# openGemini/openGemini

Hardware: NVIDIA H100
Metric: decoded+aggregated rows/s (higher is better)
Workload: dtype f64

## Files before the change

opengemini_b200/csrc/agg_kernels.cuh:

```cuda
#pragma once
#include "agg_ops.cuh"
#include "decode.cuh"
#include "internal.h"

namespace ogpu {

#define OG_NO_BUCKET 0xFFFFFFFFu

struct DirP {
    const uint8_t *data;
    const uint64_t *page_off;
    const uint32_t *page_len;
    const uint32_t *seg_series, *seg_rows, *series_seg_begin;
    const int64_t *seg_tmin, *seg_tmax;
    uint32_t n_segments, n_columns;
};

struct ChunkP {
    uint32_t series_begin, series_end;
    uint32_t seg_begin, seg_end;
    Tri cells[OG_MAX_CALLS];
    uint32_t nb;
    Tri edges[OG_MAX_CALLS];
    uint32_t *edge_bucket;
    Tri gcells[OG_MAX_CALLS];
    uint32_t gc_cols, gc_tail0, gc_edge0, gc_col0;
    uint32_t J;
    int *err;
    int *flags;
};

__device__ __forceinline__ size_t cell_idx(const ChunkP &ch, uint32_t series, uint32_t b) { return (size_t)(series - ch.series_begin) * ch.nb + b; }

__device__ __forceinline__ void report_err(int *err, int code, uint32_t seg) {
    if (atomicCAS(&err[0], 0, code) == 0) err[1] = (int)seg;
}

__device__ __forceinline__ void store_part(const Tri &a, size_t i, const Part &p) {
    a.val[i] = p.v; a.ok[i] = (uint8_t)p.ok;
    if (a.tim) a.tim[i] = p.t;
}
__device__ __forceinline__ Part load_part(const Tri &a, size_t i) {
    Part p; p.ok = a.ok[i]; p.v = a.val[i]; p.t = a.tim ? a.tim[i] : 0; return p;
}
__device__ __forceinline__ void store_cell(const ChunkP &ch, int call, uint32_t series, uint32_t b, const Part &p) {
    store_part(ch.cells[call], cell_idx(ch, series, b), p);
    ch.flags[0] = 1;
}

struct SegWindows {
    const QueryP &q; const ChunkP &ch;
    const uint32_t seg; const size_t e; const uint32_t series;
    uint32_t cur_b = OG_NO_BUCKET, head_b = OG_NO_BUCKET; bool head_done = false;
    int64_t we = 0;

    __device__ __forceinline__ SegWindows(const QueryP &q_, const ChunkP &ch_, uint32_t seg_, size_t e_, uint32_t series_)
        : q(q_), ch(ch_), seg(seg_), e(e_), series(series_) {}
    template <int NC> __device__ __forceinline__ void flush(const Part (&parts)[NC], bool final) {
        if (cur_b == OG_NO_BUCKET) return;
#pragma unroll
        for (int c = 0; c < NC; c++) {
            if (!head_done) store_part(ch.edges[c], e, parts[c]);
            else if (final) store_part(ch.edges[c], e + 1, parts[c]);
            else if (parts[c].ok) store_cell(ch, c, series, cur_b, parts[c]);
        }
        if (!head_done) { head_done = true; head_b = cur_b; }
    }
    template <int NC> __device__ __forceinline__ bool enter(int64_t t, Part (&parts)[NC]) {
        if (cur_b != OG_NO_BUCKET && t < we) return true;
        flush(parts, false);
        cur_b = bucket_of(t, q.start, q.interval);
        if (cur_b >= q.n_buckets) { report_err(ch.err, D_CORRUPT, seg); cur_b = OG_NO_BUCKET; return false; }
        we = q.start + (int64_t)(cur_b + 1) * q.interval;
#pragma unroll
        for (int c = 0; c < NC; c++) parts[c] = part_empty();
        return true;
    }
    template <int NC> __device__ __forceinline__ void end(const Part (&parts)[NC]) {
        const uint32_t last_b = cur_b;
        const bool single = !head_done;
        flush(parts, true);
        ch.edge_bucket[e] = head_b;
        ch.edge_bucket[e + 1] = (single || head_b == OG_NO_BUCKET) ? OG_NO_BUCKET : last_b;
        if (head_b != OG_NO_BUCKET) ch.flags[1] = 1;
    }
};

__global__ void k_validate(DirP d, const int32_t *col_types, uint32_t *seg_rows, unsigned long long *totals ,
                           uint32_t *max_rows, int *err) {
    uint32_t seg = blockIdx.x * blockDim.x + threadIdx.x;
    if (seg >= d.n_segments) return;
    size_t ti = (size_t)d.n_columns * d.n_segments + seg;
    TimeDesc t;
    int rc = parse_time_page(d.data + d.page_off[ti], d.page_len[ti], t);
    if (rc == D_OK && t.rows == 0) rc = D_CORRUPT;
    if (rc == D_OK) {
        int64_t last = t.t0; bool unsorted = false;
        if (t.kind == 0) last = (int64_t)((uint64_t)t.t0 + (uint64_t)(t.rows - 1) * t.delta);
        else {
            TimeIter it; it.init(t);
            for (uint32_t i = 0; i < t.rows; i++) { const int64_t x = it.next(); unsorted |= x < last; last = x; }
            it.finish(); rc = it.err;
        }
        if (rc == D_OK && (t.t0 < d.seg_tmin[seg] || last > d.seg_tmax[seg] || last < t.t0 || unsorted)) rc = D_CORRUPT;
    }
    if (rc != D_OK) { report_err(err, rc, seg); seg_rows[seg] = 0; return; }
    seg_rows[seg] = t.rows;
    unsigned long long bytes = d.page_len[ti];
    for (uint32_t c = 0; c < d.n_columns; c++) {
        size_t pi = (size_t)c * d.n_segments + seg;
        uint32_t len = d.page_len[pi];
        if (len == 0) continue;
        bytes += len;
        PageHdr h;
        rc = parse_field_header(d.data + d.page_off[pi], len, col_types[c], t.rows, h);
        if (rc == D_OK && h.rows != t.rows) rc = D_CORRUPT;
        if (rc == D_OK && h.bitmap && hdr_valid_rows(h) != h.rows - h.nil_count) rc = D_CORRUPT;
        if (rc == D_OK && !h.one_row && h.nil_count < h.rows) {
            if (h.block_len < 1) rc = D_CORRUPT;
            else {
                int tag = __ldg(h.block) >> 4, ty = col_types[c];
                if (ty == OG_TYPE_FLOAT) rc = (tag == 0 || tag == 3 || tag == 4 || tag == 5) ? D_OK : (tag == 1 || tag == 2 || tag == 6) ? D_UNSUPPORTED : D_CORRUPT;
                else if (ty == OG_TYPE_INT) rc = (tag == 1 || tag == 2 || tag == 4) ? D_OK : tag == 3 ? D_UNSUPPORTED : D_CORRUPT;
                else if (ty == OG_TYPE_BOOL) rc = tag == 1 ? D_OK : D_CORRUPT;
                else if (ty == OG_TYPE_STRING) rc = D_OK;
                else rc = D_UNSUPPORTED;
            }
        }
        if (rc != D_OK) { report_err(err, rc, seg); return; }
    }
    atomicAdd(&totals[0], (unsigned long long)t.rows);
    atomicAdd(&totals[1], bytes);
    atomicMax(max_rows, t.rows);
    if (t.kind != 0 && t.kind != 3) atomicAdd(&totals[2], 1ull);
}

__global__ void k_fill_seg_series(const uint32_t *series_seg_begin, uint32_t n_series, uint32_t *seg_series) {
    uint32_t s = blockIdx.x;
    if (s >= n_series) return;
    for (uint32_t g = series_seg_begin[s] + threadIdx.x; g < series_seg_begin[s + 1]; g += blockDim.x) seg_series[g] = s;
}

struct TileP {
    uint32_t tile_begin, tile_end, R;
    uint32_t S;
    uint64_t *vals[OG_MAX_COLS];
    uint8_t *okb[OG_MAX_COLS];
    int64_t *times;
    uint8_t *keep;
};

__global__ void k_decode_tile(DirP d, QueryP q, TileP tp, int *err) {
    uint32_t seg = tp.tile_begin + blockIdx.x * blockDim.x + threadIdx.x;
    if (seg >= tp.tile_end) return;
    uint32_t slot = blockIdx.y;
    const size_t base = seg - tp.tile_begin, S = tp.S;
    uint32_t rows = d.seg_rows[seg];
    if (slot == q.n_cols) {
        size_t ti = (size_t)d.n_columns * d.n_segments + seg;
        TimeDesc t;
        int rc = parse_time_page(d.data + d.page_off[ti], d.page_len[ti], t);
        if (rc == D_OK) {
            TimeIter it; it.init(t);
            for (uint32_t i = 0; i < t.rows; i++) tp.times[base + i * S] = it.next();
            it.finish(); rc = it.err;
        }
        if (rc != D_OK) report_err(err, rc, seg);
        return;
    }
    size_t pi = (size_t)q.col_index[slot] * d.n_segments + seg;
    uint64_t *out = tp.vals[slot] + base; uint8_t *okb = tp.okb[slot] + base;
    ColIter it;
    it.init(d.data + d.page_off[pi], d.page_len[pi], q.col_type[slot], rows);
    for (uint32_t i = 0; i < rows; i++) { uint64_t v = 0; okb[i * S] = it.next(v); out[i * S] = v; }
    it.finish();
    if (it.err != D_OK) report_err(err, it.err, seg);
}

__device__ __forceinline__ bool term_pass(const FilterP &f, uint64_t raw) {
    if (f.type == OG_TYPE_FLOAT || (f.type == OG_TYPE_INT && f.const_is_float)) {
        double v = f.type == OG_TYPE_FLOAT ? u2d(raw) : (double)(int64_t)raw;
        double c = f.const_is_float ? f.fval : (double)f.ival;
        switch (f.op) {
        case OG_OP_LT: return !(v >= c);
        case OG_OP_LTE: return !(v > c);
        case OG_OP_GT: return !(v <= c);
        case OG_OP_GTE: return !(v < c);
        case OG_OP_EQ: return !(v != c);
        default: return !(v == c);
        }
    }
    int64_t v = f.type == OG_TYPE_BOOL ? (int64_t)(raw != 0) : (int64_t)raw, c = f.ival;
    switch (f.op) {
    case OG_OP_LT: return !(v >= c);
    case OG_OP_LTE: return !(v > c);
    case OG_OP_GT: return !(v <= c);
    case OG_OP_GTE: return !(v < c);
    case OG_OP_EQ: return !(v != c);
    default: return !(v == c);
    }
}

__global__ void k_filter_tile(DirP d, QueryP q, TileP tp) {
    size_t idx = (size_t)blockIdx.x * blockDim.x + threadIdx.x;
    size_t total = (size_t)tp.S * tp.R;
    if (idx >= total) return;
    uint32_t row = (uint32_t)(idx / tp.S), sl = (uint32_t)(idx % tp.S);
    if (sl >= tp.tile_end - tp.tile_begin) return;
    if (row >= d.seg_rows[tp.tile_begin + sl]) { tp.keep[idx] = 0; return; }
    int64_t t = tp.times[idx];
    bool keep = t >= q.tmin && t <= q.tmax;
    if (keep && q.n_filter) {
        uint32_t stack = 0; int sp = 0;
        for (uint32_t i = 0; i < q.n_filter; i++) {
            const FilterP &f = q.filter[i];
            if (f.kind == OG_F_TERM) {
                bool pass = tp.okb[f.col_slot][idx] && term_pass(f, tp.vals[f.col_slot][idx]);
                stack |= (uint32_t)pass << sp; sp++;
            } else {
                uint32_t b = (stack >> (sp - 1)) & 1, a = (stack >> (sp - 2)) & 1;
                uint32_t r = f.kind == OG_F_AND ? (a & b) : (a | b);
                sp -= 2; stack &= ~(3u << sp); stack |= r << sp; sp++;
            }
        }
        keep = stack & 1;
    }
    tp.keep[idx] = keep;
}

__global__ void k_window_reduce(DirP d, QueryP q, TileP tp, ChunkP ch) {
    uint32_t sl = blockIdx.x * blockDim.x + threadIdx.x;
    uint32_t seg = tp.tile_begin + sl;
    if (seg >= tp.tile_end) return;
    const uint32_t rows = d.seg_rows[seg], series = d.seg_series[seg];
    const size_t S = tp.S, e = 2 * (size_t)(seg - ch.seg_begin);
    Part parts[OG_MAX_CALLS];
    uint32_t cur_b = OG_NO_BUCKET, head_b = OG_NO_BUCKET; bool head_done = false;
    int64_t we = 0;
    auto flush = [&](bool final) {
        if (cur_b == OG_NO_BUCKET) return;
        for (uint32_t c = 0; c < q.n_calls; c++) {
            if (!head_done) store_part(ch.edges[c], e, parts[c]);
            else if (final) store_part(ch.edges[c], e + 1, parts[c]);
            else if (parts[c].ok) store_cell(ch, (int)c, series, cur_b, parts[c]);
        }
        if (!head_done) { head_done = true; head_b = cur_b; }
    };
    for (uint32_t r = 0; r < rows; r++) {
        const size_t ix = (size_t)r * S + sl;
        const int64_t t = tp.times[ix];
        if (t < q.tmin) continue;
        if (t > q.tmax) break;
        if (cur_b == OG_NO_BUCKET || t >= we) {
            flush(false);
            cur_b = bucket_of(t, q.start, q.interval);
            if (cur_b >= q.n_buckets) { report_err(ch.err, D_CORRUPT, seg); cur_b = OG_NO_BUCKET; break; }
            we = q.start + (int64_t)(cur_b + 1) * q.interval;
#pragma unroll
            for (uint32_t c = 0; c < OG_MAX_CALLS; c++) parts[c] = part_empty();
        }
        if (!tp.keep[ix]) continue;
#pragma unroll
        for (uint32_t c = 0; c < OG_MAX_CALLS; c++) {
            if (c >= q.n_calls) break;
            const CallP &cp = q.calls[c];
            if (tp.okb[cp.col_slot][ix]) acc_row(cp.func, cp.type, parts[c], tp.vals[cp.col_slot][ix], t);
        }
    }
    flush(true);
    ch.edge_bucket[e] = head_b;
    ch.edge_bucket[e + 1] = (head_b == OG_NO_BUCKET || cur_b == head_b) ? OG_NO_BUCKET : cur_b;
}

struct EdgeRuns { uint32_t hb, tb, s_end; bool head_leader; };
__device__ __forceinline__ EdgeRuns edge_runs(const DirP &d, const ChunkP &ch, uint32_t seg, uint32_t series) {
    EdgeRuns r;
    const uint32_t s_first = d.series_seg_begin[series];
    r.s_end = d.series_seg_begin[series + 1];
    const uint32_t *eb = ch.edge_bucket;
    const size_t e = 2 * (size_t)(seg - ch.seg_begin);
    r.hb = eb[e]; r.tb = eb[e + 1];
    r.head_leader = true;
    if (r.hb != OG_NO_BUCKET && seg > s_first) {
        const size_t pe = e - 2;
        const uint32_t pb = eb[pe + 1] != OG_NO_BUCKET ? eb[pe + 1] : eb[pe];
        if (pb != OG_NO_BUCKET && pb == r.hb) r.head_leader = false;
    }
    return r;
}
__device__ __forceinline__ Part edge_stitch(const QueryP &q, const ChunkP &ch, const EdgeRuns &r, uint32_t seg, int which, uint32_t c) {
    const CallP &cp = q.calls[c];
    const uint32_t *eb = ch.edge_bucket;
    const size_t e = 2 * (size_t)(seg - ch.seg_begin);
    const uint32_t b = which == 0 ? r.hb : r.tb;
    Part acc = load_part(ch.edges[c], e + which);
    if (which == 1 || r.tb == OG_NO_BUCKET) {
        for (uint32_t nx = seg + 1; nx < r.s_end; nx++) {
            const size_t ne = 2 * (size_t)(nx - ch.seg_begin);
            if (eb[ne] != b) break;
            acc = series_merge(cp.func, cp.type, acc, load_part(ch.edges[c], ne));
            if (eb[ne + 1] != OG_NO_BUCKET) break;
        }
    }
    return acc;
}

__global__ void k_fix_edges(DirP d, QueryP q, ChunkP ch) {
    uint32_t seg = ch.seg_begin + blockIdx.x * blockDim.x + threadIdx.x;
    if (seg >= ch.seg_end) return;
    const uint32_t series = d.seg_series[seg];
    const EdgeRuns r = edge_runs(d, ch, seg, series);
    if (r.hb == OG_NO_BUCKET) return;
    for (int which = 0; which < 2; which++) {
        if (which == 0 && !r.head_leader) continue;
        if (which == 1 && r.tb == OG_NO_BUCKET) continue;
        const uint32_t b = which == 0 ? r.hb : r.tb;
        if (b >= q.n_buckets) { report_err(ch.err, D_CORRUPT, seg); continue; }
        for (uint32_t c = 0; c < q.n_calls; c++) {
            const Part acc = edge_stitch(q, ch, r, seg, which, c);
            if (acc.ok) store_cell(ch, (int)c, series, b, acc);
        }
    }
}

__device__ __forceinline__ Part shfl_xor_part(const Part &p, int o, bool with_time) {
    Part r; r.v = __shfl_xor_sync(0xffffffffu, p.v, o); r.ok = __shfl_xor_sync(0xffffffffu, p.ok, o);
    r.t = with_time ? __shfl_xor_sync(0xffffffffu, p.t, o) : 0;
    return r;
}
__device__ __forceinline__ Part warp_fold(int func, int type, bool multi, Part p, bool with_time) {
#pragma unroll
    for (int o = 16; o; o >>= 1) { const Part other = shfl_xor_part(p, o, with_time); group_update(func, type, multi, p, other); }
    return p;
}
__device__ __forceinline__ bool call_has_time(const QueryP &q, uint32_t c) { return q.calls[c].func >= OG_AGG_MIN && !(q.multi && q.calls[c].func <= OG_AGG_MAX); }
__device__ __forceinline__ int call_ftype(const QueryP &q, uint32_t c) { return q.calls[c].func == OG_AGG_COUNT ? OG_TYPE_INT : q.calls[c].type; }

__global__ void k_fix_edges_fold(DirP d, QueryP q, ChunkP ch) {
    if (ch.flags[1] == 0) return;
    const uint32_t w = (blockIdx.x * blockDim.x + threadIdx.x) >> 5, lane = threadIdx.x & 31;
    const uint32_t n_blk = (ch.series_end - ch.series_begin + 31) / 32;
    if (w >= n_blk * ch.J) return;
    const uint32_t blk = w / ch.J, j = w % ch.J;
    const uint32_t series = ch.series_begin + blk * 32 + lane;
    const bool in = series < ch.series_end;
    const uint32_t seg = in ? d.series_seg_begin[series] + j : 0;
    EdgeRuns r; r.hb = r.tb = OG_NO_BUCKET; r.head_leader = false; r.s_end = 0;
    if (in) r = edge_runs(d, ch, seg, series);
    const uint32_t n_bk = (ch.gc_cols - ch.gc_edge0) / 3;
    for (int which = 0; which < 2; which++) {
        const uint32_t gcol = ch.gc_edge0 + (which ? 2u : (j & 1u)) * n_bk + ch.series_begin / 32 + blk - ch.gc_col0;
        const bool has = r.hb != OG_NO_BUCKET && (which == 0 ? r.head_leader : r.tb != OG_NO_BUCKET);
        const uint32_t b = which == 0 ? r.hb : r.tb;
        const uint32_t hm = __ballot_sync(0xffffffffu, has);
        if (hm == 0) continue;
        const int leader = __ffs(hm) - 1;
        const uint32_t bL = __shfl_sync(0xffffffffu, b, leader);
        const bool unif = __all_sync(0xffffffffu, !has || b == bL) && bL < q.n_buckets;
        if (!unif && has && b >= q.n_buckets) { report_err(ch.err, D_CORRUPT, seg); continue; }
        for (uint32_t c = 0; c < q.n_calls; c++) {
            Part acc = part_empty();
            if (has) acc = edge_stitch(q, ch, r, seg, which, c);
            if (unif) {
                acc = warp_fold(q.calls[c].func, call_ftype(q, c), q.multi != 0, acc, call_has_time(q, c));
                if ((int)lane == leader && acc.ok) store_part(ch.gcells[c], (size_t)bL * ch.gc_cols + gcol, acc);
            } else if (has && acc.ok) store_cell(ch, (int)c, series, b, acc);
        }
    }
}

struct GroupP {
    const uint32_t *grp_begin;
    const uint32_t *grp_series;
    uint32_t n_groups;
    Tri dense[OG_MAX_CALLS];
};

__global__ void k_merge_groups(QueryP q, ChunkP ch, GroupP gp) {
    if (ch.flags[0] == 0) return;
    size_t idx = (size_t)blockIdx.x * blockDim.x + threadIdx.x;
    size_t total = (size_t)gp.n_groups * q.n_buckets;
    if (idx >= total) return;
    uint32_t g = (uint32_t)(idx / q.n_buckets), b = (uint32_t)(idx % q.n_buckets);
    uint32_t lo = gp.grp_begin[g], hi = gp.grp_begin[g + 1];
    {
        uint32_t a = lo, z = hi;
        while (a < z) { uint32_t m = (a + z) >> 1; if (gp.grp_series[m] < ch.series_begin) a = m + 1; else z = m; }
        lo = a;
    }
    if (lo >= hi || gp.grp_series[lo] >= ch.series_end) return;
    {
        const uint32_t c = blockIdx.y;
        const CallP &cp = q.calls[c];
        Part acc = load_part(gp.dense[c], idx);
        const Tri cells = ch.cells[c];
        constexpr int U = 16;
        for (uint32_t i = lo; i < hi; i += U) {
            uint32_t okv[U]; uint64_t vv[U]; int64_t tt[U];
#pragma unroll
            for (int u = 0; u < U; u++) {
                uint32_t ii = i + u;
                uint32_t s = ii < hi ? gp.grp_series[ii] : 0xffffffffu;
                bool in = s < ch.series_end;
                size_t ci = in ? cell_idx(ch, s, b) : 0;
                okv[u] = in ? cells.ok[ci] : 0;
                vv[u] = okv[u] ? cells.val[ci] : 0;
                tt[u] = (okv[u] && cells.tim) ? cells.tim[ci] : 0;
            }
#pragma unroll
            for (int u = 0; u < U; u++) {
                if (!okv[u]) continue;
                Part p; p.ok = 1; p.v = vv[u]; p.t = tt[u];
                group_update(cp.func, cp.out_type == OG_TYPE_INT && cp.func == OG_AGG_COUNT ? OG_TYPE_INT : cp.type, q.multi != 0, acc, p);
            }
        }
        store_part(gp.dense[c], idx, acc);
    }
}

__global__ void k_merge_per_series(QueryP q, ChunkP ch, GroupP gp) {
    const uint32_t c = blockIdx.y;
    const size_t n = (size_t)(ch.series_end - ch.series_begin) * q.n_buckets;
    const size_t i = (size_t)blockIdx.x * blockDim.x + threadIdx.x;
    if (i >= n) return;
    const CallP &cp = q.calls[c];
    const int ftype = cp.out_type == OG_TYPE_INT && cp.func == OG_AGG_COUNT ? OG_TYPE_INT : cp.type;
    const uint32_t b = (uint32_t)(i % q.n_buckets);
    Part p; p.ok = ch.cells[c].ok[i]; p.v = p.ok ? ch.cells[c].val[i] : 0; p.t = (p.ok && ch.cells[c].tim) ? ch.cells[c].tim[i] : 0;
    Part a; a.v = 0; a.ok = 0; a.t = q.multi ? 0 : q.start + (int64_t)b * q.interval;
    group_update(cp.func, ftype, q.multi != 0, a, p);
    store_part(gp.dense[c], (size_t)ch.series_begin * q.n_buckets + i, a);
}

#define OG_MERGE_SB 256u
__global__ void __launch_bounds__(128) k_merge_all_blocks(QueryP q, ChunkP ch, GroupP gp) {
    if (ch.flags[0] == 0) return;
    const uint32_t b = blockIdx.x * blockDim.x + threadIdx.x, blk = blockIdx.y, c = blockIdx.z;
    if (b >= q.n_buckets) return;
    const uint32_t nS = ch.series_end - ch.series_begin;
    const uint32_t s0 = blk * OG_MERGE_SB, s1 = min(nS, s0 + OG_MERGE_SB);
    const int func = q.calls[c].func, ftype = call_ftype(q, c);
    const bool multi = q.multi != 0;
    const Tri cells = ch.cells[c];
    Part acc = part_empty();
    constexpr int U = 8;
    for (uint32_t s = s0; s < s1; s += U) {
        uint32_t okv[U]; uint64_t vv[U]; int64_t tt[U];
#pragma unroll
        for (int u = 0; u < U; u++) {
            const bool in = s + u < s1;
            const size_t ci = in ? (size_t)(s + u) * ch.nb + b : 0;
            okv[u] = in ? cells.ok[ci] : 0;
            vv[u] = okv[u] ? cells.val[ci] : 0;
            tt[u] = (okv[u] && cells.tim) ? cells.tim[ci] : 0;
        }
#pragma unroll
        for (int u = 0; u < U; u++) {
            if (!okv[u]) continue;
            Part p; p.ok = 1; p.v = vv[u]; p.t = tt[u];
            group_update(func, ftype, multi, acc, p);
        }
    }
    if (acc.ok) store_part(ch.gcells[c], (size_t)b * ch.gc_cols + blk, acc);
}

__global__ void k_merge_folded(QueryP q, ChunkP ch, GroupP gp) {
    const uint32_t b = (blockIdx.x * blockDim.x + threadIdx.x) >> 5, lane = threadIdx.x & 31, c = blockIdx.y;
    if (b >= q.n_buckets) return;
    const int func = q.calls[c].func, ftype = call_ftype(q, c);
    const bool wt = call_has_time(q, c), multi = q.multi != 0;
    const Tri g = ch.gcells[c];
    Part acc = part_empty();
    const size_t row = (size_t)b * ch.gc_cols;
    for (uint32_t col = lane; col < ch.gc_cols; col += 32) {
        if (!g.ok[row + col]) continue;
        Part p; p.ok = 1; p.v = g.val[row + col]; p.t = wt ? g.tim[row + col] : 0;
        group_update(func, ftype, multi, acc, p);
    }
    acc = warp_fold(func, ftype, multi, acc, wt);
    if (lane == 0 && acc.ok) {
        Part a = load_part(gp.dense[c], b);
        group_update(func, ftype, multi, a, acc);
        store_part(gp.dense[c], b, a);
    }
}

__global__ void k_init_dense(QueryP q, GroupP gp) {
    size_t idx = (size_t)blockIdx.x * blockDim.x + threadIdx.x;
    size_t total = (size_t)gp.n_groups * q.n_buckets;
    if (idx >= total) return;
    uint32_t b = (uint32_t)(idx % q.n_buckets);
    for (uint32_t c = 0; c < q.n_calls; c++) {
        gp.dense[c].val[idx] = 0; gp.dense[c].ok[idx] = 0;
        if (gp.dense[c].tim) gp.dense[c].tim[idx] = q.multi ? 0 : q.start + (int64_t)b * q.interval;
    }
}

__global__ void k_merge_dense(QueryP q, GroupP mine, GroupP other) {
    size_t idx = (size_t)blockIdx.x * blockDim.x + threadIdx.x;
    size_t total = (size_t)mine.n_groups * q.n_buckets;
    if (idx >= total) return;
    for (uint32_t c = 0; c < q.n_calls; c++) {
        const CallP &cp = q.calls[c];
        Part a = load_part(mine.dense[c], idx), p = load_part(other.dense[c], idx);
        group_update(cp.func, cp.func == OG_AGG_COUNT ? OG_TYPE_INT : cp.type, q.multi != 0, a, p);
        store_part(mine.dense[c], idx, a);
    }
}

}
```

opengemini_b200/csrc/api.cu:

```cuda
#include <algorithm>
#include <cstdarg>
#include <cstdio>
#include <cstring>
#include <numeric>

#include "agg_kernels.cuh"
#include "il_build.cuh"
#include "fused_multi.cuh"
#include "fused_cols.cuh"
#include "snappy_load.cuh"
#include <cub/device/device_scan.cuh>
#include <cub/device/device_radix_sort.cuh>
#include "internal.h"

namespace ogpu {

static thread_local char g_err[512] = "";
void set_error(const char *fmt, ...) {
    va_list ap; va_start(ap, fmt); vsnprintf(g_err, sizeof g_err, fmt, ap); va_end(ap);
}
int cuda_fail(cudaError_t e, const char *what, const char *file, int line) {
    set_error("CUDA error %d (%s) at %s:%d: %s", (int)e, cudaGetErrorString(e), file, line, what);
    return OG_E_CUDA;
}
static int g_device = -1;
cudaError_t dev_mem_info(size_t *free_b, size_t *total_b) {
    cudaError_t e = cudaMemGetInfo(free_b, total_b);
    if (e != cudaSuccess) return e;
    cudaMemPool_t pool; uint64_t reserved = 0, used = 0; int dev = 0;
    if (cudaGetDevice(&dev) == cudaSuccess && cudaDeviceGetDefaultMemPool(&pool, dev) == cudaSuccess &&
        cudaMemPoolGetAttribute(pool, cudaMemPoolAttrReservedMemCurrent, &reserved) == cudaSuccess &&
        cudaMemPoolGetAttribute(pool, cudaMemPoolAttrUsedMemCurrent, &used) == cudaSuccess && reserved > used) *free_b += (size_t)(reserved - used);
    else cudaGetLastError();
    return cudaSuccess;
}

static int map_dev_err(int code) {
    switch (code) {
    case D_UNSUPPORTED: return OG_E_UNSUPPORTED;
    case D_TYPE: return OG_E_TYPE;
    case D_WATCHDOG: return OG_E_CUDA;
    default: return OG_E_CORRUPT;
    }
}

static DirP make_dir(const og_shard *s) {
    DirP d;
    d.data = s->d_data; d.page_off = s->d_page_off; d.page_len = s->d_page_len; d.seg_series = s->d_seg_series;
    d.seg_rows = s->d_seg_rows; d.series_seg_begin = s->d_series_seg_begin; d.seg_tmin = s->d_tmin; d.seg_tmax = s->d_tmax;
    d.n_segments = s->n_segments; d.n_columns = s->n_columns;
    return d;
}

int shard_finalize(og_shard *s, bool scan_snappy) {
    int rc;
    s->il.resize(s->n_columns);
    if ((rc = dalloc(&s->d_seg_series, s->n_segments))) return rc;
    if ((rc = dalloc(&s->d_seg_rows, s->n_segments))) return rc;
    Scratch tmp;
    int32_t *d_types; unsigned long long *d_tot; uint32_t *d_max; int *d_err;
    if ((rc = tmp.get(&d_types, s->n_columns)) || (rc = tmp.get(&d_tot, 3)) || (rc = tmp.get(&d_max, 1)) || (rc = tmp.get(&d_err, 2))) return rc;
    CU(cudaMemcpy(d_types, s->col_types.data(), s->n_columns * sizeof(int32_t), cudaMemcpyHostToDevice));
    CU(cudaMemset(d_tot, 0, 24)); CU(cudaMemset(d_max, 0, 4)); CU(cudaMemset(d_err, 0, 8));
    if (s->n_series) k_fill_seg_series<<<s->n_series, 128>>>(s->d_series_seg_begin, s->n_series, s->d_seg_series);
    if (s->n_segments && scan_snappy) {
        const size_t n_pages = (size_t)(s->n_columns + 1) * s->n_segments;
        Scratch tr;
        uint32_t *tr_size; unsigned long long *d_cnt;
        if ((rc = tr.get(&tr_size, n_pages)) || (rc = tr.get(&d_cnt, 3))) return rc;
        CU(cudaMemset(d_cnt, 0, 24));
        k_snappy_scan<<<(s->n_segments + 127) / 128, 128>>>(make_dir(s), d_types, tr_size, d_cnt);
        unsigned long long cnt[3];
        CU(cudaMemcpy(cnt, d_cnt, 24, cudaMemcpyDeviceToHost));
        if (cnt[0]) {
            if (!s->owns_data) { set_error("shard has %llu Snappy pages: they are transcoded at open, which needs a library-owned copy of the data (do not pass OG_SHARD_DEVICE_DATA)", cnt[0]); return OG_E_UNSUPPORTED; }
            uint64_t *tr_off; uint8_t *scan_tmp; size_t tb = 0;
            if ((rc = tr.get(&tr_off, n_pages))) return rc;
            CU(cub::DeviceScan::ExclusiveSum(nullptr, tb, tr_size, tr_off, (int)n_pages));
            if ((rc = tr.get(&scan_tmp, tb))) return rc;
            CU(cub::DeviceScan::ExclusiveSum(scan_tmp, tb, tr_size, tr_off, (int)n_pages));
            const uint64_t new_base = (s->data_len + 15) & ~15ull, new_len = new_base + cnt[2];
            const DirP loaded = make_dir(s);
            uint8_t *nd;
            if ((rc = dalloc(&nd, (size_t)new_len + 1024))) return rc;
            tr.bufs.push_back(s->d_data); s->d_data = nd;
            CU(cudaMemcpy(nd, loaded.data, s->data_len, cudaMemcpyDeviceToDevice));
            CU(cudaMemset(nd + s->data_len, 0, new_len + 1024 - s->data_len));
            k_snappy_transcode<<<(unsigned)((n_pages + 127) / 128), 128>>>(loaded, tr_size, tr_off, nd, new_base, s->d_page_off, s->d_page_len, d_err);
            CU(cudaGetLastError());
            CU(cudaDeviceSynchronize());
            s->data_len = new_len;
            s->snappy_pages = cnt[0]; s->snappy_bytes_in = cnt[1]; s->snappy_bytes_out = cnt[2];
        }
    }
    if (s->n_segments) k_validate<<<(s->n_segments + 127) / 128, 128>>>(make_dir(s), d_types, s->d_seg_rows, d_tot, d_max, d_err);
    CU(cudaGetLastError());
    unsigned long long tot[3]; int err[2]; uint32_t mx;
    CU(cudaMemcpy(tot, d_tot, 24, cudaMemcpyDeviceToHost));
    CU(cudaMemcpy(err, d_err, 8, cudaMemcpyDeviceToHost));
    CU(cudaMemcpy(&mx, d_max, 4, cudaMemcpyDeviceToHost));
    if (err[0]) {
        set_error("segment %d: %s page (device validation code %d)", err[1], err[0] == D_UNSUPPORTED ? "unsupported codec in" : err[0] == D_TYPE ? "type mismatch in" : "corrupt", err[0]);
        return map_dev_err(err[0]);
    }
    s->n_rows = tot[0]; s->page_bytes = tot[1] - s->snappy_bytes_out + s->snappy_bytes_in;
    s->max_seg_rows = mx; s->irregular_time_pages = tot[2];
    return OG_OK;
}

int alloc_dir(og_shard *s) {
    const size_t nseg = s->n_segments, n_pages = ((size_t)s->n_columns + 1) * nseg;
    int rc;
    if ((rc = dalloc(&s->d_series_seg_begin, (size_t)s->n_series + 1)) || (rc = dalloc(&s->d_tmin, nseg)) || (rc = dalloc(&s->d_tmax, nseg)) ||
        (rc = dalloc(&s->d_page_off, n_pages)) || (rc = dalloc(&s->d_page_len, n_pages)) || (rc = dalloc(&s->d_sids, (size_t)s->n_series)))
        return rc;
    return OG_OK;
}

int upload_dir(og_shard *s, const uint32_t *series_seg_begin, const int64_t *seg_tmin, const int64_t *seg_tmax, const uint64_t *page_off,
               const uint32_t *page_len, const uint64_t *sids) {
    int rc = alloc_dir(s); if (rc) return rc;
    const size_t nseg = s->n_segments, n_pages = ((size_t)s->n_columns + 1) * nseg;
    CU(cudaMemcpy(s->d_series_seg_begin, series_seg_begin, ((size_t)s->n_series + 1) * 4, cudaMemcpyHostToDevice));
    CU(cudaMemcpy(s->d_tmin, seg_tmin, nseg * 8, cudaMemcpyHostToDevice));
    CU(cudaMemcpy(s->d_tmax, seg_tmax, nseg * 8, cudaMemcpyHostToDevice));
    CU(cudaMemcpy(s->d_page_off, page_off, n_pages * 8, cudaMemcpyHostToDevice));
    CU(cudaMemcpy(s->d_page_len, page_len, n_pages * 4, cudaMemcpyHostToDevice));
    CU(cudaMemcpy(s->d_sids, sids, (size_t)s->n_series * 8, cudaMemcpyHostToDevice));
    return OG_OK;
}

}

using namespace ogpu;

extern "C" {

OG_API int og_device_count(void) { int n = 0; if (cudaGetDeviceCount(&n) != cudaSuccess) return 0; return n; }

OG_API int og_init(int device_ordinal) {
    int n = og_device_count();
    if (n <= 0) { set_error("no CUDA device visible: libogpu has no CPU path"); return OG_E_CUDA; }
    if (device_ordinal < 0 || device_ordinal >= n) { set_error("device ordinal %d out of range (%d devices)", device_ordinal, n); return OG_E_INVAL; }
    CU(cudaSetDevice(device_ordinal));
    CU(cudaFree(0));
    {
        cudaMemPool_t pool; uint64_t thr = ~0ull;
        if (cudaDeviceGetDefaultMemPool(&pool, device_ordinal) == cudaSuccess) cudaMemPoolSetAttribute(pool, cudaMemPoolAttrReleaseThreshold, &thr);
        else cudaGetLastError();
    }
    g_device = device_ordinal;
    return OG_OK;
}

OG_API const char *og_strerror(int st) {
    switch (st) {
    case OG_OK: return "ok";
    case OG_EOF: return "end of stream";
    case OG_E_INVAL: return "invalid argument";
    case OG_E_CUDA: return "CUDA failure or no device bound";
    case OG_E_NOMEM: return "out of device memory";
    case OG_E_UNSUPPORTED: return "unsupported codec or option on the GPU path";
    case OG_E_CORRUPT: return "corrupt page";
    case OG_E_ABORTED: return "query aborted";
    case OG_E_TYPE: return "column type mismatch";
    case OG_E_STATE: return "call sequence error";
    default: return "unknown status";
    }
}
OG_API const char *og_last_error(void) { return g_err; }
OG_API const char *og_version(void) { return "ogpu 0.2 (sm_90a)"; }
OG_API int og_release_cached_memory(void) {
    if (g_device < 0) return OG_OK;
    CU(cudaSetDevice(g_device));
    CU(cudaDeviceSynchronize());
    cudaMemPool_t pool;
    CU(cudaDeviceGetDefaultMemPool(&pool, g_device));
    CU(cudaMemPoolTrimTo(pool, 0));
    return OG_OK;
}

}
namespace ogpu {
int ensure_device() {
    if (g_device < 0) { int rc = og_init(0); if (rc != OG_OK) return rc; }
    else CU(cudaSetDevice(g_device));
    return OG_OK;
}
}
static int need_device() { return ogpu::ensure_device(); }
extern "C" {

OG_API void og_shard_close(og_shard *s) { delete s; }

}
namespace ogpu {
int check_desc(const og_shard_desc *d) {
    if (d->n_columns > 64 || (d->n_segments && (!d->seg_tmin || !d->seg_tmax || !d->time_page_off || !d->time_page_len)) || (d->n_series && !d->series_seg_begin)) { set_error("bad shard descriptor"); return OG_E_INVAL; }
    for (uint32_t s = 0; s < d->n_series; s++) if (d->series_seg_begin[s] > d->series_seg_begin[s + 1]) { set_error("series_seg_begin not monotone at %u", s); return OG_E_INVAL; }
    if (d->n_series && d->series_seg_begin[d->n_series] != d->n_segments) { set_error("series_seg_begin[n_series] != n_segments"); return OG_E_INVAL; }
    for (uint32_t c = 0; c < d->n_columns; c++)
        if (d->columns[c].type != OG_TYPE_INT && d->columns[c].type != OG_TYPE_FLOAT && d->columns[c].type != OG_TYPE_BOOL && d->columns[c].type != OG_TYPE_STRING) {
            set_error("column %u: unknown column type %d", c, d->columns[c].type); return OG_E_UNSUPPORTED;
        }
    for (size_t c = 0; c <= d->n_columns; c++) {
        const uint64_t *po = c < d->n_columns ? d->columns[c].page_off : d->time_page_off;
        const uint32_t *pl = c < d->n_columns ? d->columns[c].page_len : d->time_page_len;
        for (size_t g = 0; g < d->n_segments; g++)
            if (po[g] + pl[g] > d->data_len) { set_error("column %zu segment %zu: page [%llu,+%u) outside data (%llu bytes)", c, g, (unsigned long long)po[g], pl[g], (unsigned long long)d->data_len); return OG_E_INVAL; }
    }
    for (uint32_t sr = 0; sr < d->n_series; sr++)
        for (uint32_t g = d->series_seg_begin[sr]; g < d->series_seg_begin[sr + 1]; g++)
            if (d->seg_tmin[g] > d->seg_tmax[g] || (g > d->series_seg_begin[sr] && d->seg_tmin[g] <= d->seg_tmax[g - 1])) {
                set_error("series %u: segment %u is not time-ordered (only ordered TSSP files are supported)", sr, g); return OG_E_UNSUPPORTED;
            }
    return OG_OK;
}
}
extern "C" {

OG_API int og_shard_open(const og_shard_desc *d, og_shard **out) {
    if (!d || !out) { set_error("null argument"); return OG_E_INVAL; }
    *out = nullptr;
    int rc = need_device(); if (rc) return rc;
    if ((rc = check_desc(d))) return rc;
    std::unique_ptr<og_shard> s(new og_shard);
    s->device = g_device; s->n_series = d->n_series; s->n_segments = d->n_segments; s->n_columns = d->n_columns;
    s->data_len = d->data_len;
    for (uint32_t c = 0; c < d->n_columns; c++) {
        s->col_types.push_back(d->columns[c].type);
        s->col_names.push_back(d->columns[c].name ? d->columns[c].name : "");
    }
    s->sids.assign(d->sids, d->sids + d->n_series);
    s->h_series_seg_begin.assign(d->series_seg_begin, d->series_seg_begin + d->n_series + 1);
    size_t nseg = d->n_segments, ncol1 = (size_t)d->n_columns + 1;
    std::vector<uint64_t> off(ncol1 * nseg); std::vector<uint32_t> len(ncol1 * nseg);
    for (size_t c = 0; c < ncol1; c++) {
        const uint64_t *po = c < d->n_columns ? d->columns[c].page_off : d->time_page_off;
        const uint32_t *pl = c < d->n_columns ? d->columns[c].page_len : d->time_page_len;
        for (size_t g = 0; g < nseg; g++) { off[c * nseg + g] = po[g]; len[c * nseg + g] = pl[g]; }
    }
    s->tmin = INT64_MAX; s->tmax = INT64_MIN;
    if (d->n_series)
        for (uint32_t g = d->series_seg_begin[0]; g < d->series_seg_begin[d->n_series]; g++) { s->tmin = std::min(s->tmin, d->seg_tmin[g]); s->tmax = std::max(s->tmax, d->seg_tmax[g]); }
    if (d->flags & OG_SHARD_DEVICE_DATA) { s->d_data = (uint8_t *)d->data; s->owns_data = false; }
    else {
        if ((rc = dalloc(&s->d_data, d->data_len + 1024))) return rc;
        CU(cudaMemcpy(s->d_data, d->data, d->data_len, cudaMemcpyHostToDevice));
        CU(cudaMemset(s->d_data + d->data_len, 0, 1024));
    }
    if ((rc = upload_dir(s.get(), d->series_seg_begin, d->seg_tmin, d->seg_tmax, off.data(), len.data(), d->sids))) return rc;
    if ((rc = shard_finalize(s.get(), true))) return rc;
    *out = s.release();
    return OG_OK;
}

OG_API int og_shard_info(const og_shard *s, uint64_t *n_series, uint64_t *n_segments, uint64_t *n_rows, uint64_t *page_bytes, int64_t *tmin, int64_t *tmax) {
    if (!s) return OG_E_INVAL;
    if (n_series) *n_series = s->n_series;
    if (n_segments) *n_segments = s->n_segments;
    if (n_rows) *n_rows = s->n_rows;
    if (page_bytes) *page_bytes = s->page_bytes;
    if (tmin) *tmin = s->tmin;
    if (tmax) *tmax = s->tmax;
    return OG_OK;
}

OG_API int og_shard_layout_get(const og_shard *s, og_shard_layout *out) {
    if (!s || !out) return OG_E_INVAL;
    out->data_len = s->data_len; out->n_series = s->n_series; out->n_segments = s->n_segments; out->n_columns = s->n_columns;
    return OG_OK;
}

OG_API int og_shard_export(const og_shard *s, uint8_t *data, uint64_t *sids, uint32_t *series_seg_begin, int64_t *seg_tmin,
                           int64_t *seg_tmax, uint64_t *page_off, uint32_t *page_len, int32_t *col_types) {
    if (!s) return OG_E_INVAL;
    CU(cudaSetDevice(s->device));
    size_t nseg = s->n_segments, ncol1 = (size_t)s->n_columns + 1;
    if (data) CU(cudaMemcpy(data, s->d_data, s->data_len, cudaMemcpyDeviceToHost));
    if (sids) memcpy(sids, s->sids.data(), s->sids.size() * 8);
    if (series_seg_begin) memcpy(series_seg_begin, s->h_series_seg_begin.data(), s->h_series_seg_begin.size() * 4);
    if (seg_tmin) CU(cudaMemcpy(seg_tmin, s->d_tmin, nseg * 8, cudaMemcpyDeviceToHost));
    if (seg_tmax) CU(cudaMemcpy(seg_tmax, s->d_tmax, nseg * 8, cudaMemcpyDeviceToHost));
    if (page_off) CU(cudaMemcpy(page_off, s->d_page_off, ncol1 * nseg * 8, cudaMemcpyDeviceToHost));
    if (page_len) CU(cudaMemcpy(page_len, s->d_page_len, ncol1 * nseg * 4, cudaMemcpyDeviceToHost));
    if (col_types) memcpy(col_types, s->col_types.data(), s->col_types.size() * 4);
    return OG_OK;
}

static const int64_t MIN_TIME = INT64_MIN + 2, MAX_TIME = INT64_MAX - 1;
static void window_of(int64_t interval, int64_t offset, int64_t tmin, int64_t tmax, int64_t t, int64_t *s, int64_t *e) {
    if (interval == 0) { *s = tmin; *e = tmax + 1; return; }
    t -= offset;
    int64_t dt = t % interval;
    if (dt < 0) dt += interval;
    int64_t st = ((int64_t)((uint64_t)MIN_TIME + (uint64_t)dt) >= t) ? MIN_TIME : t - dt;
    st += offset;
    int64_t d2 = interval - dt;
    int64_t en = (MAX_TIME - d2 <= t) ? MAX_TIME : t + d2;
    en += offset;
    *s = st; *e = en;
}
static bool window_clamped(int64_t interval, int64_t offset, int64_t t) {
    const __int128 x = (__int128)t - offset;
    __int128 r = x % interval;
    if (r < 0) r += interval;
    const __int128 s = x - r, e = s + interval;
    return s < MIN_TIME || e > MAX_TIME || s + offset < INT64_MIN || e + offset > INT64_MAX;
}

}
namespace { void free_plan(void *plan); }
extern "C" void og_query_free_merge_state(void *p);
og_query::~og_query() {
    if (stream) cudaStreamSynchronize(stream);
    if (live) { std::lock_guard<std::mutex> lock(live->mu); live->n--; }
    og_query_free_merge_state(merge_state);
    free_plan(plan);
    if (ev0) cudaEventDestroy(ev0);
    if (ev1) cudaEventDestroy(ev1);
    for (cudaEvent_t e : main_ev) cudaEventDestroy(e);
    if (stream) cudaStreamDestroy(stream);
}
extern "C" {
OG_API void og_query_destroy(og_query *q) { delete q; }

OG_API int og_query_create(og_shard *s, const og_query_desc *d_in, og_query **out) {
    if (!s || !d_in || !out) { set_error("null argument"); return OG_E_INVAL; }
    *out = nullptr;
    og_query_desc d_clamped = *d_in;
    d_clamped.tmin = std::max(d_in->tmin, MIN_TIME); d_clamped.tmax = std::min(d_in->tmax, MAX_TIME);
    const og_query_desc *d = &d_clamped;
    CU(cudaSetDevice(s->device));
    if (d->n_calls == 0 || d->n_calls > OG_MAX_CALLS) { set_error("n_calls must be 1..%d", OG_MAX_CALLS); return OG_E_INVAL; }
    if (d->n_filter > OG_MAX_FILTER) { set_error("filter too long (max %d items)", OG_MAX_FILTER); return OG_E_INVAL; }
    if (d->interval < 0 || d->tmin > d->tmax) { set_error("bad interval or time range"); return OG_E_INVAL; }
    std::unique_ptr<og_query> q(new og_query);
    {
        std::lock_guard<std::mutex> lock(s->live->mu);
        s->live->n++;
        q->sh = s; q->live = s->live;
    }
    q->desc = *d;
    q->calls.assign(d->calls, d->calls + d->n_calls);
    if (d->n_filter) q->filter.assign(d->filter, d->filter + d->n_filter);
    q->desc.calls = q->calls.data(); q->desc.filter = q->filter.data();
    QueryP &p = q->qp;
    memset(&p, 0, sizeof p);
    auto slot_of = [&](int col) -> int {
        for (uint32_t i = 0; i < p.n_cols; i++) if (p.col_index[i] == col) return (int)i;
        if (p.n_cols >= OG_MAX_COLS) return -1;
        p.col_index[p.n_cols] = col; p.col_type[p.n_cols] = s->col_types[col];
        return (int)p.n_cols++;
    };
    for (uint32_t i = 0; i < d->n_calls; i++) {
        const og_call &c = d->calls[i];
        if (c.column < 0 || (uint32_t)c.column >= s->n_columns || c.func < OG_AGG_COUNT || c.func > OG_AGG_LAST) { set_error("call %u: bad column or function", i); return OG_E_INVAL; }
        int type = s->col_types[c.column];
        if (type == OG_TYPE_STRING && c.func != OG_AGG_COUNT) { set_error("call %u: only count() is pushed down for string columns (their values are never decoded on the GPU path)", i); return OG_E_UNSUPPORTED; }
        if (c.func == OG_AGG_SUM && type == OG_TYPE_BOOL) { set_error("sum() over a boolean column (unsupported sum iterator type, series_call_processor.go:140)"); return OG_E_INVAL; }
        int sl = slot_of(c.column);
        if (sl < 0) { set_error("too many distinct columns"); return OG_E_INVAL; }
        p.calls[i].func = c.func; p.calls[i].col_slot = sl; p.calls[i].type = type;
        p.calls[i].out_type = c.func == OG_AGG_COUNT ? OG_TYPE_INT : type;
    }
    p.n_calls = d->n_calls; p.multi = d->n_calls > 1;
    int sp = 0;
    for (uint32_t i = 0; i < d->n_filter; i++) {
        const og_filter_item &f = d->filter[i];
        FilterP &fp = p.filter[i];
        fp.kind = f.kind;
        if (f.kind == OG_F_TERM) {
            if (f.column < 0 || (uint32_t)f.column >= s->n_columns || f.op < OG_OP_LT || f.op > OG_OP_NEQ) { set_error("filter item %u: bad column or op", i); return OG_E_INVAL; }
            if (s->col_types[f.column] == OG_TYPE_STRING) { set_error("filter item %u: WHERE on a string column is not pushed down", i); return OG_E_UNSUPPORTED; }
            int sl = slot_of(f.column);
            if (sl < 0) { set_error("too many distinct columns"); return OG_E_INVAL; }
            fp.col_slot = sl; fp.op = f.op; fp.type = s->col_types[f.column]; fp.const_is_float = f.const_is_float; fp.fval = f.fval; fp.ival = f.ival;
            sp++;
        } else if (f.kind == OG_F_AND || f.kind == OG_F_OR) {
            if (sp < 2) { set_error("filter RPN underflow at item %u", i); return OG_E_INVAL; }
            sp--;
        } else { set_error("filter item %u: bad kind", i); return OG_E_INVAL; }
    }
    if (d->n_filter && sp != 1) { set_error("filter RPN does not reduce to one value"); return OG_E_INVAL; }
    p.n_filter = d->n_filter;
    int64_t gmin = std::max(d->tmin, s->tmin), gmax = std::min(d->tmax, s->tmax);
    bool overlap = gmin <= gmax;
    if (!overlap) gmin = gmax = d->tmin;
    if (d->flags & OG_Q_QUERY_GRID) {
        if (d_in->tmin <= MIN_TIME || d_in->tmax >= MAX_TIME) { set_error("OG_Q_QUERY_GRID needs a bounded time range"); return OG_E_INVAL; }
        gmin = d->tmin; gmax = d->tmax; overlap = true;
    }
    int64_t s0, e0, s1, e1;
    if (d->interval == 0) { s0 = gmin; e0 = gmax + 1; s1 = s0; e1 = e0; }
    else {
        if (overlap && (window_clamped(d->interval, d->offset, gmin) || window_clamped(d->interval, d->offset, gmax))) {
            set_error("the first or last window of the range is clamped at the int64 time limits"); return OG_E_UNSUPPORTED;
        }
        window_of(d->interval, d->offset, d->tmin, d->tmax, gmin, &s0, &e0);
        window_of(d->interval, d->offset, d->tmin, d->tmax, gmax + 1, &s1, &e1);
    }
    p.tmin = d->tmin; p.tmax = d->tmax; p.start = s0; p.interval = e0 - s0;
    if (p.interval <= 0) { set_error("degenerate window"); return OG_E_INVAL; }
    uint64_t nb = d->interval ? (uint64_t)(e1 - s0) / (uint64_t)p.interval : 1;
    if (nb == 0 || nb > 0x7fffffffull) { set_error("query range yields %llu buckets", (unsigned long long)nb); return OG_E_INVAL; }
    p.n_buckets = (uint32_t)nb;
    q->n_groups = d->group_mode == OG_GROUP_ALL ? 1 : d->group_mode == OG_GROUP_PER_SERIES ? s->n_series : d->n_groups;
    if (d->group_mode == OG_GROUP_MAP) {
        if (!d->series_group || d->n_groups == 0) { set_error("OG_GROUP_MAP needs series_group and n_groups"); return OG_E_INVAL; }
        q->series_group.assign(d->series_group, d->series_group + s->n_series);
        for (uint32_t g : q->series_group) if (g >= d->n_groups) { set_error("series_group entry out of range"); return OG_E_INVAL; }
    } else if (d->group_mode != OG_GROUP_ALL && d->group_mode != OG_GROUP_PER_SERIES) { set_error("bad group_mode"); return OG_E_INVAL; }
    if (q->n_groups == 0) q->n_groups = 1;
    cudaError_t e = cudaStreamCreateWithFlags(&q->stream, cudaStreamNonBlocking);
    if (e != cudaSuccess) return cuda_fail(e, "cudaStreamCreate", __FILE__, __LINE__);
    cudaEventCreate(&q->ev0); cudaEventCreate(&q->ev1);
    *out = q.release();
    return OG_OK;
}

OG_API void og_query_abort(og_query *q) { if (q) q->aborted = 1; }

}
namespace {
struct Plan {
    ChunkP ch; TileP tp; GroupP gp;
    bool fused;
    bool cols;
    bool multi;
    bool fast;
    bool blockmerge;
    bool fold;
    int fm; bool times;
    IlP il;
    const og_shard::IlCol *ic;
};
void free_plan(void *plan) { delete (Plan *)plan; }

template <int NC> void launch_fused(const DirP &d, const QueryP &p, const ChunkP &ch, const uint32_t *list, uint32_t n, cudaStream_t st) {
    if (n) k_fused_segment<NC><<<(n + 127) / 128, 128, 0, st>>>(d, p, ch, list, n);
}
template <int FM, bool TIMES> void launch_fast_t(bool fold, const IlP &il, uint32_t g0, uint32_t g1, const QueryP &p, const ChunkP &ch, cudaStream_t st) {
    constexpr uint32_t WPB = OG_FAST_THREADS / 32;
    dim3 grid((g1 - g0 + WPB - 1) / WPB), block(OG_FAST_THREADS);
    if (fold) k_fused_il<FM, TIMES, true><<<grid, block, WPB * il_acc_bytes(p.n_calls, TIMES), st>>>(p, ch, il, g0, g1);
    else k_fused_il<FM, TIMES, false><<<grid, block, 0, st>>>(p, ch, il, g0, g1);
}
void launch_fast(int fm, bool times, bool fold, const IlP &il, uint32_t g0, uint32_t g1, const QueryP &p, const ChunkP &ch, cudaStream_t st) {
    if (g1 <= g0) return;
    if (!times) {
        switch (fm) {
        case FM_SUM | FM_COUNT: return launch_fast_t<FM_SUM | FM_COUNT, false>(fold, il, g0, g1, p, ch, st);
        case FM_SUM | FM_COUNT | FM_MAX: return launch_fast_t<FM_SUM | FM_COUNT | FM_MAX, false>(fold, il, g0, g1, p, ch, st);
        case FM_SUM | FM_COUNT | FM_MIN | FM_MAX: return launch_fast_t<FM_SUM | FM_COUNT | FM_MIN | FM_MAX, false>(fold, il, g0, g1, p, ch, st);
        case FM_COUNT: return launch_fast_t<FM_COUNT, false>(fold, il, g0, g1, p, ch, st);
        default: break;
        }
    } else {
        switch (fm) {
        case FM_MAX | FM_COUNT: return launch_fast_t<FM_MAX | FM_COUNT, true>(fold, il, g0, g1, p, ch, st);
        case FM_MIN | FM_COUNT: return launch_fast_t<FM_MIN | FM_COUNT, true>(fold, il, g0, g1, p, ch, st);
        default: break;
        }
    }
    return launch_fast_t<63, true>(fold, il, g0, g1, p, ch, st);
}

template <int NCOL, int NCALL> void launch_multi_t(const QueryP &p, const DirP &d, const ChunkP &ch, uint32_t nseg, cudaStream_t st) {
    bool simple = true;
    for (uint32_t c = 0; c < p.n_calls; c++) simple &= p.calls[c].func == OG_AGG_COUNT || p.calls[c].func == OG_AGG_SUM;
    const unsigned gb = (nseg + 127) / 128;
    if (simple) k_fused_multi<NCOL, NCALL, true><<<gb, 128, 0, st>>>(d, p, ch);
    else k_fused_multi<NCOL, NCALL, false><<<gb, 128, 0, st>>>(d, p, ch);
}
template <int NCOL> void launch_multi_c(const QueryP &p, const DirP &d, const ChunkP &ch, uint32_t nseg, cudaStream_t st) {
    switch (p.n_calls) {
    case 1: return launch_multi_t<NCOL, 1>(p, d, ch, nseg, st);
    case 2: return launch_multi_t<NCOL, 2>(p, d, ch, nseg, st);
    case 3: return launch_multi_t<NCOL, 3>(p, d, ch, nseg, st);
    case 4: return launch_multi_t<NCOL, 4>(p, d, ch, nseg, st);
    case 5: return launch_multi_t<NCOL, 5>(p, d, ch, nseg, st);
    case 6: return launch_multi_t<NCOL, 6>(p, d, ch, nseg, st);
    case 7: return launch_multi_t<NCOL, 7>(p, d, ch, nseg, st);
    default: return launch_multi_t<NCOL, 8>(p, d, ch, nseg, st);
    }
}
void launch_cols(const QueryP &p, const DirP &d, const ChunkP &ch, uint32_t nseg, cudaStream_t st) {
    bool simple = true;
    for (uint32_t c = 0; c < p.n_calls; c++) simple &= p.calls[c].func == OG_AGG_COUNT || p.calls[c].func == OG_AGG_SUM;
    const unsigned gb = (nseg + 127) / 128;
    if (simple) k_fused_cols<true><<<gb, 128, 0, st>>>(d, p, ch);
    else k_fused_cols<false><<<gb, 128, 0, st>>>(d, p, ch);
}
void launch_multi(const QueryP &p, const DirP &d, const ChunkP &ch, uint32_t nseg, cudaStream_t st) {
    switch (p.n_cols) {
    case 1: return launch_multi_c<1>(p, d, ch, nseg, st);
    case 2: return launch_multi_c<2>(p, d, ch, nseg, st);
    case 3: return launch_multi_c<3>(p, d, ch, nseg, st);
#ifdef OG_WIDE_MULTI
    case 5: return launch_multi_c<5>(p, d, ch, nseg, st);
    case 6: return launch_multi_c<6>(p, d, ch, nseg, st);
    case 7: return launch_multi_c<7>(p, d, ch, nseg, st);
    case 8: return launch_multi_c<8>(p, d, ch, nseg, st);
#endif
    default: return launch_multi_c<4>(p, d, ch, nseg, st);
    }
}

int ensure_il(og_shard *s, int col, cudaStream_t st) {
    std::lock_guard<std::mutex> lock(s->il_mu);
    if (s->il.size() != s->n_columns) s->il.resize(s->n_columns);
    og_shard::IlCol &ic = s->il[col];
    if (ic.state != 0) return OG_OK;
    ic.state = -1;
    if (s->n_segments == 0 || s->col_types[col] != OG_TYPE_FLOAT) return OG_OK;
    const uint32_t nseg = s->n_segments;
    uint32_t J = s->n_series ? s->h_series_seg_begin[1] - s->h_series_seg_begin[0] : 0;
    for (uint32_t i = 0; i < s->n_series && J; i++) if (s->h_series_seg_begin[i + 1] - s->h_series_seg_begin[i] != J) J = 0;
    const uint32_t n_super = J ? (s->n_series + OG_IL_SUPER - 1) / OG_IL_SUPER : 1;
    const uint64_t n_dom64 = J ? (uint64_t)n_super * J : 1;
    if (n_dom64 >= (1ull << 31)) return OG_OK;
    const uint32_t n_dom = (uint32_t)n_dom64;
    int rc;
    struct Ev { cudaEvent_t e = nullptr; Ev() { cudaEventCreate(&e); } ~Ev() { if (e) cudaEventDestroy(e); } } ev0, ev1;
    cudaEventRecord(ev0.e, st);
    Scratch tmp(st);
    IlScanOut so{};
    uint32_t *seg_words; uint64_t *keys2; uint32_t *vals2;
    if ((rc = tmp.get(&so.seg_win, nseg)) || (rc = tmp.get(&so.n_packed, 1)) ||
        (rc = tmp.get(&seg_words, nseg)) || (rc = tmp.get(&so.seg_t0, nseg)) || (rc = tmp.get(&so.seg_dt, nseg)) || (rc = tmp.get(&so.keys, nseg)) ||
        (rc = tmp.get(&so.vals, nseg)) || (rc = tmp.get(&keys2, nseg)) || (rc = tmp.get(&vals2, nseg)) || (rc = tmp.get(&so.dom_cnt, n_dom))) return rc;
    so.seg_words = seg_words;
    if ((rc = tmp.get(&so.misaligned, 1))) return rc;
    CU(cudaMemsetAsync(so.dom_cnt, 0, (size_t)n_dom * 4, st));
    CU(cudaMemsetAsync(so.misaligned, 0, 4, st));
    CU(cudaMemsetAsync(so.n_packed, 0, 8, st));
    DirP d = make_dir(s);
    k_il_scan<<<(nseg + 255) / 256, 256, 0, st>>>(d, col, s->col_types[col], J, so);
    CU(cudaGetLastError());
    int dbits = 1; while ((1ull << dbits) < n_dom64 + 1) dbits++;
    {
        size_t tb = 0;
        CU(cub::DeviceRadixSort::SortPairs(nullptr, tb, so.keys, keys2, so.vals, vals2, (int)nseg, 0, (int)OG_IL_WORD_BITS + dbits, st));
        void *dtmp; if ((rc = tmp.get((uint8_t **)&dtmp, tb))) return rc;
        CU(cub::DeviceRadixSort::SortPairs(dtmp, tb, so.keys, keys2, so.vals, vals2, (int)nseg, 0, (int)OG_IL_WORD_BITS + dbits, st));
    }
    std::vector<uint32_t> dom_cnt(n_dom); uint32_t misaligned = 1; unsigned long long n_packed = 0;
    CU(cudaMemcpyAsync(dom_cnt.data(), so.dom_cnt, (size_t)n_dom * 4, cudaMemcpyDeviceToHost, st));
    CU(cudaMemcpyAsync(&misaligned, so.misaligned, 4, cudaMemcpyDeviceToHost, st));
    CU(cudaMemcpyAsync(&n_packed, so.n_packed, 8, cudaMemcpyDeviceToHost, st));
    CU(cudaStreamSynchronize(st));
    std::vector<uint32_t> elem_first(n_dom), grp_first(n_dom);
    uint64_t n_elig = 0, ng64 = 0;
    for (uint32_t i = 0; i < n_dom; i++) { elem_first[i] = (uint32_t)n_elig; grp_first[i] = (uint32_t)ng64; n_elig += dom_cnt[i]; ng64 += (dom_cnt[i] + 31) / 32; }
    const uint32_t n_gen = nseg - (uint32_t)n_elig;
    if (n_gen) {
        if ((rc = dalloc(&ic.gen_list, (size_t)n_gen))) return rc;
        CU(cudaMemcpyAsync(ic.gen_list, vals2 + n_elig, (size_t)n_gen * 4, cudaMemcpyDeviceToDevice, st));
        ic.gen_host.resize(n_gen);
        CU(cudaMemcpyAsync(ic.gen_host.data(), vals2 + n_elig, (size_t)n_gen * 4, cudaMemcpyDeviceToHost, st));
        CU(cudaStreamSynchronize(st));
    }
    if (n_elig == 0) return OG_OK;
    const uint32_t ng = (uint32_t)ng64;
    ic.n_groups = ng; ic.J = J; ic.aligned = J != 0 && misaligned == 0; ic.n_super = n_super; ic.cols_per_super = OG_IL_SUPER / 32 + 1;
    ic.super_grp_first.assign(n_super + 1, ng);
    for (uint32_t sp = 0; sp < n_super; sp++) ic.super_grp_first[sp] = grp_first[J ? sp * J : 0];
    uint32_t *d_elem_first, *d_grp_first;
    if ((rc = tmp.get(&d_elem_first, n_dom)) || (rc = tmp.get(&d_grp_first, n_dom))) return rc;
    CU(cudaMemcpyAsync(d_elem_first, elem_first.data(), (size_t)n_dom * 4, cudaMemcpyHostToDevice, st));
    CU(cudaMemcpyAsync(d_grp_first, grp_first.data(), (size_t)n_dom * 4, cudaMemcpyHostToDevice, st));
    const size_t n_slots = (size_t)ng * 32;
    if ((rc = dalloc(&ic.lane_seg, n_slots)) || (rc = dalloc(&ic.lane_rows, n_slots)) || (rc = dalloc(&ic.lane_win, n_slots)) || (rc = dalloc(&ic.lane_series, n_slots)) ||
        (rc = dalloc(&ic.lane_t0, n_slots)) || (rc = dalloc(&ic.lane_dt, n_slots)) || (rc = dalloc(&ic.grp_col, (size_t)ng)) ||
        (rc = dalloc(&ic.grp_rows, (size_t)ng)) || (rc = dalloc(&ic.grp_off, (size_t)ng))) return rc;
    CU(cudaMemsetAsync(ic.lane_seg, 0xff, n_slots * 4, st));
    CU(cudaMemsetAsync(ic.lane_rows, 0, n_slots * 4, st));
    CU(cudaMemsetAsync(ic.lane_win, 0, n_slots * 2, st));
    IlAssign as{};
    as.keys = keys2; as.segs = vals2; as.elem_first = d_elem_first; as.grp_first = d_grp_first;
    as.seg_words = seg_words; as.seg_t0 = so.seg_t0; as.seg_dt = so.seg_dt; as.seg_win = so.seg_win;
    as.lane_seg = ic.lane_seg; as.lane_rows = ic.lane_rows; as.lane_series = ic.lane_series; as.grp_col = ic.grp_col; as.lane_win = ic.lane_win; as.lane_t0 = ic.lane_t0; as.lane_dt = ic.lane_dt;
    as.n_elig = (uint32_t)n_elig; as.J = J; as.cols_per_super = ic.cols_per_super;
    k_il_assign<<<(unsigned)((n_elig + 255) / 256), 256, 0, st>>>(d, as);
    k_il_group_rows<<<(unsigned)((n_slots + 255) / 256), 256, 0, st>>>(ng, ic.lane_seg, seg_words, ic.grp_rows);
    CU(cudaGetLastError());
    std::vector<uint32_t> gw(ng); std::vector<uint64_t> go(ng);
    CU(cudaMemcpyAsync(gw.data(), ic.grp_rows, (size_t)ng * 4, cudaMemcpyDeviceToHost, st));
    CU(cudaStreamSynchronize(st));
    uint64_t total = 0;
    for (uint32_t g = 0; g < ng; g++) { go[g] = total; total += (uint64_t)gw[g] * 32; }
    size_t free_b = 0, total_b = 0;
    CU(dev_mem_info(&free_b, &total_b));
    size_t headroom = (size_t)8 << 30;
    if (const char *ov = getenv("OGPU_IL_HEADROOM_MB")) headroom = (size_t)atoll(ov) << 20;
    if (total * 4 + headroom > free_b || dev_malloc((void **)&ic.words, total * 4) != cudaSuccess) {
        cudaGetLastError(); ic.words = nullptr; ic.state = -2;
        return OG_OK;
    }
    CU(cudaMemcpyAsync(ic.grp_off, go.data(), (size_t)ng * 8, cudaMemcpyHostToDevice, st));
    k_il_repack<<<(unsigned)((n_slots + 127) / 128), 128, 0, st>>>(d, col, ic.lane_seg, ic.lane_win, ic.grp_off, ic.grp_rows, ng, ic.words);
    CU(cudaGetLastError());
    cudaEventRecord(ev1.e, st);
    CU(cudaStreamSynchronize(st));
    float ms = 0; cudaEventElapsedTime(&ms, ev0.e, ev1.e);
    ic.n_words = total; ic.n_packed = n_packed; ic.build_ms = ms; ic.state = 1;
    return OG_OK;
}

int build_plan(og_query *q) {
    og_shard *s = q->sh;
    const QueryP &p = q->qp;
    cudaStream_t st = q->stream;
    int rc;
    Plan *pl = new Plan;
    memset((void *)pl, 0, sizeof *pl);
    q->plan = pl;
    size_t cells_dense = (size_t)q->n_groups * p.n_buckets;
    for (uint32_t c = 0; c < p.n_calls; c++) {
        bool sel = p.calls[c].func >= OG_AGG_MIN && !(p.multi && p.calls[c].func <= OG_AGG_MAX);
        if ((rc = q->bufs.get(&q->dense[c].val, cells_dense))) return rc;
        if ((rc = q->bufs.get(&q->dense[c].ok, cells_dense))) return rc;
        if (sel && (rc = q->bufs.get(&q->dense[c].tim, cells_dense))) return rc;
    }
    std::vector<uint32_t> grp_begin(q->n_groups + 1, 0), grp_series(s->n_series);
    if (q->desc.group_mode == OG_GROUP_MAP) {
        for (uint32_t sr = 0; sr < s->n_series; sr++) grp_begin[q->series_group[sr] + 1]++;
        for (uint32_t g = 0; g < q->n_groups; g++) grp_begin[g + 1] += grp_begin[g];
        std::vector<uint32_t> cur(grp_begin.begin(), grp_begin.end() - 1);
        for (uint32_t sr = 0; sr < s->n_series; sr++) grp_series[cur[q->series_group[sr]]++] = sr;
    } else if (q->desc.group_mode == OG_GROUP_PER_SERIES) {
        for (uint32_t g = 0; g <= q->n_groups; g++) grp_begin[g] = std::min(g, s->n_series);
        std::iota(grp_series.begin(), grp_series.end(), 0u);
    } else { grp_begin[1] = s->n_series; std::iota(grp_series.begin(), grp_series.end(), 0u); }
    uint32_t *d_grp_begin, *d_grp_series;
    if ((rc = q->bufs.get(&d_grp_begin, grp_begin.size()))) return rc;
    if ((rc = q->bufs.get(&d_grp_series, grp_series.size()))) return rc;
    if ((rc = q->bufs.get(&q->d_err, 16))) return rc;
    CU(cudaMemcpyAsync(d_grp_begin, grp_begin.data(), grp_begin.size() * 4, cudaMemcpyHostToDevice, st));
    CU(cudaMemcpyAsync(d_grp_series, grp_series.data(), grp_series.size() * 4, cudaMemcpyHostToDevice, st));
    CU(cudaStreamSynchronize(st));
    pl->gp.grp_begin = d_grp_begin; pl->gp.grp_series = d_grp_series; pl->gp.n_groups = q->n_groups;
    for (uint32_t c = 0; c < p.n_calls; c++) pl->gp.dense[c] = q->dense[c];

    bool has_string = false;
    for (uint32_t k = 0; k < p.n_cols; k++) has_string |= p.col_type[k] == OG_TYPE_STRING;
    pl->fused = p.n_cols == 1 && p.n_filter == 0 && !has_string && !(q->desc.flags & OG_Q_NO_FUSED);
    const bool multi_ok = !pl->fused && (has_string || !(q->desc.flags & OG_Q_NO_FUSED));
    pl->cols = false;
    if (multi_ok && !(q->desc.flags & OG_Q_NO_FAST) && s->irregular_time_pages == 0 && s->max_seg_rows <= OG_COLS_MAXROWS &&
        (p.n_filter == 0 || (p.n_filter == 1 && p.filter[0].kind == OG_F_TERM)) && !getenv("OGPU_NO_COLS")) {
        pl->cols = true;
        for (uint32_t k = 0; k < p.n_cols; k++) {
            int n = 0;
            for (uint32_t c = 0; c < p.n_calls; c++) n += p.calls[c].col_slot == (int)k;
            if (n > OG_COLS_MAXMINE) pl->cols = false;
        }
    }
    if (has_string && !pl->cols && p.n_cols > OG_MULTI_MAXC) { set_error("a query that counts a string column may touch at most %d columns on this shard", OG_MULTI_MAXC); return OG_E_UNSUPPORTED; }
    pl->multi = pl->cols || (multi_ok && p.n_cols <= OG_MULTI_MAXC);
    q->path_used = pl->fused ? 1 : pl->cols ? 5 : pl->multi ? 4 : 0;
    const bool want_fast = pl->fused && p.col_type[0] == OG_TYPE_FLOAT && !(q->desc.flags & OG_Q_NO_FAST) && s->n_segments;
    if (want_fast && (rc = ensure_il(s, p.col_index[0], st))) return rc;
    pl->fast = want_fast && s->il[p.col_index[0]].state == 1;
    const og_shard::IlCol *ic = pl->fast ? &s->il[p.col_index[0]] : nullptr;
    pl->ic = ic;
    pl->fold = pl->fast && ic->J != 0 && ic->aligned && q->desc.group_mode == OG_GROUP_ALL && !(q->desc.flags & OG_Q_STRICT_ORDER);

    size_t cell_bytes_per_series = 0;
    for (uint32_t c = 0; c < p.n_calls; c++) cell_bytes_per_series += (size_t)p.n_buckets * (9 + (p.calls[c].func >= OG_AGG_MIN ? 8 : 0));
    size_t free_b = 0, total_b = 0;
    CU(dev_mem_info(&free_b, &total_b));
    size_t budget = std::min<size_t>(free_b / 3, (size_t)24 << 30);
    q->chunk_series = (uint32_t)std::max<size_t>(1, std::min<size_t>(s->n_series, budget / std::max<size_t>(1, cell_bytes_per_series)));
    if (const char *ov = getenv("OGPU_CHUNK_SERIES")) {
        long v = atol(ov);
        if (v > 0) q->chunk_series = (uint32_t)std::min<long>(v, (long)std::max<uint32_t>(1, s->n_series));
    }
    if (q->chunk_series < s->n_series) {
        if (q->chunk_series >= OG_IL_SUPER) q->chunk_series = q->chunk_series / OG_IL_SUPER * OG_IL_SUPER;
        else q->chunk_series = std::max<uint32_t>(32, q->chunk_series & ~31u);
    }
    uint32_t max_chunk_segs = 0;
    for (uint32_t a = 0; a < s->n_series; a += q->chunk_series) {
        uint32_t b = std::min(s->n_series, a + q->chunk_series);
        max_chunk_segs = std::max(max_chunk_segs, s->h_series_seg_begin[b] - s->h_series_seg_begin[a]);
    }
    ChunkP &ch = pl->ch;
    ch.err = q->d_err; ch.flags = q->d_err + 2;
    ch.nb = p.n_buckets;
    ch.J = ic ? ic->J : 0;
    size_t chunk_cells = (size_t)std::min(q->chunk_series, s->n_series) * p.n_buckets;
    for (uint32_t c = 0; c < p.n_calls; c++) {
        bool sel = p.calls[c].func >= OG_AGG_MIN;
        if ((rc = q->bufs.get(&ch.cells[c].val, chunk_cells))) return rc;
        if ((rc = q->bufs.get(&ch.cells[c].ok, chunk_cells))) return rc;
        if (sel && (rc = q->bufs.get(&ch.cells[c].tim, chunk_cells))) return rc;
        if ((rc = q->bufs.get(&ch.edges[c].val, 2 * (size_t)max_chunk_segs))) return rc;
        if ((rc = q->bufs.get(&ch.edges[c].ok, 2 * (size_t)max_chunk_segs))) return rc;
        if (sel && (rc = q->bufs.get(&ch.edges[c].tim, 2 * (size_t)max_chunk_segs))) return rc;
    }
    if ((rc = q->bufs.get(&ch.edge_bucket, 2 * (size_t)max_chunk_segs))) return rc;
    pl->blockmerge = !pl->fold && q->desc.group_mode == OG_GROUP_ALL && !(q->desc.flags & OG_Q_STRICT_ORDER) &&
                     (s->n_series > 2 * OG_MERGE_SB || getenv("OGPU_FORCE_BLOCKMERGE") );
    if (pl->blockmerge) {
        ch.gc_edge0 = 0; ch.gc_col0 = 0;
        ch.gc_cols = (std::min(q->chunk_series, s->n_series) + OG_MERGE_SB - 1) / OG_MERGE_SB;
        const size_t n = (size_t)p.n_buckets * ch.gc_cols;
        for (uint32_t c = 0; c < p.n_calls; c++) {
            bool sel = p.calls[c].func >= OG_AGG_MIN;
            if ((rc = q->bufs.get(&ch.gcells[c].val, n))) return rc;
            if ((rc = q->bufs.get(&ch.gcells[c].ok, n))) return rc;
            if (sel && (rc = q->bufs.get(&ch.gcells[c].tim, n))) return rc;
        }
    }
    if (pl->fold) {
        ch.gc_tail0 = ic->n_super * ic->cols_per_super; ch.gc_edge0 = 2 * ch.gc_tail0; ch.gc_col0 = 0;
        ch.gc_cols = ch.gc_edge0 + 3 * ((s->n_series + 31) / 32);
        const size_t n = (size_t)p.n_buckets * ch.gc_cols;
        for (uint32_t c = 0; c < p.n_calls; c++) {
            bool sel = p.calls[c].func >= OG_AGG_MIN;
            if ((rc = q->bufs.get(&ch.gcells[c].val, n))) return rc;
            if ((rc = q->bufs.get(&ch.gcells[c].ok, n))) return rc;
            if (sel && (rc = q->bufs.get(&ch.gcells[c].tim, n))) return rc;
        }
    }
    if (pl->fast) {
        pl->il.words = ic->words; pl->il.grp_off = ic->grp_off; pl->il.grp_rows = ic->grp_rows; pl->il.grp_col = ic->grp_col;
        pl->il.lane_seg = ic->lane_seg; pl->il.lane_rows = ic->lane_rows; pl->il.lane_win = ic->lane_win; pl->il.lane_series = ic->lane_series; pl->il.lane_t0 = ic->lane_t0; pl->il.lane_dt = ic->lane_dt;
        pl->fm = 0; pl->times = false;
        for (uint32_t c = 0; c < p.n_calls; c++) {
            pl->fm |= 1 << (p.calls[c].func - 1);
            if (p.calls[c].func >= OG_AGG_MIN && !(p.multi && p.calls[c].func <= OG_AGG_MAX)) pl->times = true;
        }
        pl->fm |= FM_COUNT;
        q->path_used = pl->fold ? 3 : 2;
    }
    if (!pl->fused && !pl->multi) {
        TileP &tp = pl->tp;
        tp.R = std::max<uint32_t>(1, s->max_seg_rows);
        size_t per_seg = (size_t)tp.R * (p.n_cols * 9 + 8 + 1);
        size_t fb = 0, tb = 0;
        CU(dev_mem_info(&fb, &tb));
        const size_t tile_budget = std::max<size_t>((size_t)96 << 20, std::min<size_t>(fb / 4, (size_t)12 << 30));
        q->tile_segs = (uint32_t)std::max<size_t>(1, std::min<size_t>(std::max<uint32_t>(1, max_chunk_segs), tile_budget / per_seg));
        q->tile_segs = std::max<uint32_t>(32, q->tile_segs & ~31u);
        tp.S = q->tile_segs;
        for (uint32_t k = 0; k < p.n_cols; k++) {
            if ((rc = q->bufs.get(&tp.vals[k], (size_t)q->tile_segs * tp.R))) return rc;
            if ((rc = q->bufs.get(&tp.okb[k], (size_t)q->tile_segs * tp.R))) return rc;
        }
        if ((rc = q->bufs.get(&tp.times, (size_t)q->tile_segs * tp.R))) return rc;
        if ((rc = q->bufs.get(&tp.keep, (size_t)q->tile_segs * tp.R))) return rc;
    }
    q->planned = true;
    return OG_OK;
}
}
extern "C" {

OG_API int og_query_run(og_query *q) {
    if (!q) return OG_E_INVAL;
    og_shard *s = q->sh;
    CU(cudaSetDevice(s->device));
    const QueryP &p = q->qp;
    cudaStream_t st = q->stream;
    int rc;
    q->host_ready = false; q->next_group = 0; q->next_row = 0;
    if (!q->planned) {
        if (q->plan) { set_error("query plan failed earlier"); return OG_E_STATE; }
        if ((rc = build_plan(q))) return rc;
    }
    Plan *pl = (Plan *)q->plan;
    ChunkP ch = pl->ch; TileP tp = pl->tp; const GroupP &gp = pl->gp;
    size_t cells_dense = (size_t)q->n_groups * p.n_buckets;
    DirP dir = make_dir(s);
    uint32_t launches = 0, n_chunks = (s->n_series + q->chunk_series - 1) / q->chunk_series;
    while (q->main_ev.size() < 2 * (size_t)n_chunks) { cudaEvent_t e; CU(cudaEventCreate(&e)); q->main_ev.push_back(e); }
    CU(cudaMemsetAsync(q->d_err, 0, 64, st));
    CU(cudaEventRecord(q->ev0, st));
    const bool per_series = q->desc.group_mode == OG_GROUP_PER_SERIES;
    if (!per_series || s->n_series == 0) { k_init_dense<<<(unsigned)((cells_dense + 255) / 256), 256, 0, st>>>(p, gp); launches++; }
    const bool clear_cells = !pl->fold || q->cells_dirty || n_chunks > 1;
    uint64_t segs_scanned = 0; uint32_t ci = 0, chunks_run = 0;
    for (uint32_t a = 0; a < s->n_series; a += q->chunk_series, ci++) {
        if (q->aborted) { cudaStreamSynchronize(st); set_error("query aborted"); return OG_E_ABORTED; }
        uint32_t b = std::min(s->n_series, a + q->chunk_series);
        ch.series_begin = a; ch.series_end = b;
        ch.seg_begin = s->h_series_seg_begin[a]; ch.seg_end = s->h_series_seg_begin[b];
        uint32_t nseg = ch.seg_end - ch.seg_begin;
        const size_t chunk_cells = (size_t)(b - a) * p.n_buckets;
        if (nseg == 0) {
            if (per_series) {
                for (uint32_t c = 0; c < p.n_calls; c++) CU(cudaMemsetAsync(ch.cells[c].ok, 0, chunk_cells, st));
                k_merge_per_series<<<dim3((unsigned)((chunk_cells + 255) / 256), p.n_calls), 256, 0, st>>>(p, ch, gp);
                launches++;
            }
            continue;
        }
        segs_scanned += nseg;
        if (clear_cells) for (uint32_t c = 0; c < p.n_calls; c++) CU(cudaMemsetAsync(ch.cells[c].ok, 0, chunk_cells, st));
        if (pl->fold || pl->blockmerge) for (uint32_t c = 0; c < p.n_calls; c++) CU(cudaMemsetAsync(ch.gcells[c].ok, 0, (size_t)p.n_buckets * ch.gc_cols, st));
        if (pl->fold && ci > 0) CU(cudaMemsetAsync(ch.flags + 1, 0, sizeof(int), st));
        CU(cudaEventRecord(q->main_ev[2 * chunks_run], st));
        if (pl->fused) {
            const uint32_t *gl = nullptr; uint32_t gn = nseg;
            if (pl->fast) {
                const og_shard::IlCol &ic = *pl->ic;
                uint32_t g0 = 0, g1 = ic.n_groups;
                if (ic.J) { g0 = ic.super_grp_first[a / OG_IL_SUPER]; g1 = ic.super_grp_first[std::min<uint32_t>(ic.n_super, (b + OG_IL_SUPER - 1) / OG_IL_SUPER)]; }
                launch_fast(pl->fm, pl->times, pl->fold, pl->il, g0, g1, p, ch, st); launches++;
                auto lo = std::lower_bound(ic.gen_host.begin(), ic.gen_host.end(), ch.seg_begin);
                auto hi = std::lower_bound(ic.gen_host.begin(), ic.gen_host.end(), ch.seg_end);
                gl = ic.gen_list + (lo - ic.gen_host.begin()); gn = (uint32_t)(hi - lo);
            }
            if (gn) {
                switch (p.n_calls) {
                case 1: launch_fused<1>(dir, p, ch, gl, gn, st); break;
                case 2: launch_fused<2>(dir, p, ch, gl, gn, st); break;
                case 3: launch_fused<3>(dir, p, ch, gl, gn, st); break;
                case 4: launch_fused<4>(dir, p, ch, gl, gn, st); break;
                case 5: launch_fused<5>(dir, p, ch, gl, gn, st); break;
                case 6: launch_fused<6>(dir, p, ch, gl, gn, st); break;
                case 7: launch_fused<7>(dir, p, ch, gl, gn, st); break;
                default: launch_fused<8>(dir, p, ch, gl, gn, st); break;
                }
                launches++;
            }
        } else if (pl->cols) {
            launch_cols(p, dir, ch, nseg, st);
        } else if (pl->multi) {
            launch_multi(p, dir, ch, nseg, st);
            launches++;
        } else {
            for (uint32_t t0 = ch.seg_begin; t0 < ch.seg_end; t0 += q->tile_segs) {
                tp.tile_begin = t0; tp.tile_end = std::min(ch.seg_end, t0 + q->tile_segs);
                uint32_t n = tp.tile_end - tp.tile_begin;
                dim3 g((n + 127) / 128, p.n_cols + 1);
                k_decode_tile<<<g, 128, 0, st>>>(dir, p, tp, q->d_err);
                size_t rows_total = (size_t)tp.S * tp.R;
                k_filter_tile<<<(unsigned)((rows_total + 255) / 256), 256, 0, st>>>(dir, p, tp);
                k_window_reduce<<<(n + 127) / 128, 128, 0, st>>>(dir, p, tp, ch);
                launches += 3;
            }
        }
        CU(cudaEventRecord(q->main_ev[2 * chunks_run + 1], st));
        chunks_run++;
        if (pl->fold) k_fix_edges_fold<<<(unsigned)(((size_t)((b - a + 31) / 32) * ch.J * 32 + 127) / 128), 128, 0, st>>>(dir, p, ch);
        else k_fix_edges<<<(nseg + 127) / 128, 128, 0, st>>>(dir, p, ch);
        if (per_series) k_merge_per_series<<<dim3((unsigned)((chunk_cells + 255) / 256), p.n_calls), 256, 0, st>>>(p, ch, gp);
        else if (pl->blockmerge) k_merge_all_blocks<<<dim3((p.n_buckets + 127) / 128, (b - a + OG_MERGE_SB - 1) / OG_MERGE_SB, p.n_calls), 128, 0, st>>>(p, ch, gp);
        else k_merge_groups<<<dim3((unsigned)((cells_dense + 127) / 128), p.n_calls), 128, 0, st>>>(p, ch, gp);
        launches += 2;
        if (pl->fold || pl->blockmerge) { k_merge_folded<<<dim3((unsigned)(((size_t)p.n_buckets * 32 + 127) / 128), p.n_calls), 128, 0, st>>>(p, ch, gp); launches++; }
    }
    CU(cudaEventRecord(q->ev1, st));
    CU(cudaGetLastError());
    CU(cudaStreamSynchronize(st));
    int err[16];
    CU(cudaMemcpy(err, q->d_err, 64, cudaMemcpyDeviceToHost));
    if (getenv("OGPU_IL_STATS")) {
        unsigned long long wait, life, pro, epi;
        memcpy(&wait, err + 8, 8); memcpy(&life, err + 10, 8); memcpy(&pro, err + 12, 8); memcpy(&epi, err + 14, 8);
        const double pc = life ? 100.0 / (double)life : 0.0;
        fprintf(stderr, "[ogpu] fused rounds: common %d rare %d (lanes not resident in %d, sit-outs %d); warp cycles: %llu waiting for batches of %llu (%.1f %%), "
                "prologue %llu (%.1f %%), epilogue %llu (%.1f %%)\n",
                err[4], err[5], err[6], err[7], wait, life, pc * (double)wait, pro, pc * (double)pro, epi, pc * (double)epi);
    }
    q->cells_dirty = err[2] != 0;
    if (err[0]) { set_error("segment %d failed to decode (device code %d)", err[1], err[0]); return map_dev_err(err[0]); }
    float ms = 0; cudaEventElapsedTime(&ms, q->ev0, q->ev1);
    double main_ms = 0;
    for (uint32_t i = 0; i < chunks_run; i++) { float m = 0; cudaEventElapsedTime(&m, q->main_ev[2 * i], q->main_ev[2 * i + 1]); main_ms += m; }
    og_stats &stt = q->stats;
    uint64_t keep_pb = stt.page_bytes, keep_rows = stt.rows_decoded, keep_segs = stt.segments_scanned;
    memset(&stt, 0, sizeof stt);
    stt.kernel_ms = ms; stt.main_kernel_ms = main_ms; stt.kernel_launches = launches; stt.path = q->path_used;
    stt.page_bytes = keep_pb; stt.rows_decoded = keep_pb ? keep_rows : s->n_rows; stt.segments_scanned = keep_pb ? keep_segs : segs_scanned;
    stt.dir_bytes = (uint64_t)segs_scanned * 32;
    stt.out_bytes = 0;
    for (uint32_t c = 0; c < p.n_calls; c++) stt.out_bytes += cells_dense * (9 + (q->dense[c].tim ? 8 : 0));
    if (p.n_cols == 1 && p.col_type[0] == OG_TYPE_FLOAT) {
        std::lock_guard<std::mutex> il_lock(s->il_mu);
        if (p.col_index[0] < (int)s->il.size()) {
            const og_shard::IlCol &ic = s->il[p.col_index[0]];
            stt.il_state = ic.state; stt.il_build_ms = ic.build_ms; stt.il_bytes = ic.n_words * 4; stt.il_packed_segments = ic.state == 1 ? ic.n_packed : 0;
            stt.general_segments = ic.state == 1 ? (uint64_t)ic.gen_host.size() : s->n_segments;
        }
    }
    stt.per_series_cells_used = err[2] != 0;
    q->ran = true;
    return OG_OK;
}

OG_API int og_query_dense(og_query *q, og_dense_view *out) {
    if (!q || !out) return OG_E_INVAL;
    if (!q->ran) { set_error("og_query_dense before og_query_run"); return OG_E_STATE; }
    const QueryP &p = q->qp;
    out->n_groups = q->n_groups; out->n_buckets = p.n_buckets; out->start = q->desc.interval ? p.start : 0; out->interval = q->desc.interval ? p.interval : 0;
    out->n_cols = p.n_calls;
    for (uint32_t c = 0; c < p.n_calls; c++) {
        q->dense_cols[c].values = q->dense[c].val; q->dense_cols[c].valid = q->dense[c].ok; q->dense_cols[c].times = q->dense[c].tim;
        q->dense_cols[c].type = p.calls[c].out_type; q->dense_cols[c].func = p.calls[c].func;
    }
    out->cols = q->dense_cols; out->stream = q->stream;
    return OG_OK;
}

}
namespace {
__global__ void k_sum_page_bytes(DirP d, QueryP q, int64_t tmin, int64_t tmax, unsigned long long *out ) {
    uint32_t seg = blockIdx.x * blockDim.x + threadIdx.x;
    if (seg >= d.n_segments) return;
    if (d.seg_tmax[seg] < tmin || d.seg_tmin[seg] > tmax) return;
    unsigned long long b = d.page_len[(size_t)d.n_columns * d.n_segments + seg];
    for (uint32_t k = 0; k < q.n_cols; k++) b += d.page_len[(size_t)q.col_index[k] * d.n_segments + seg];
    atomicAdd(&out[0], b); atomicAdd(&out[1], (unsigned long long)d.seg_rows[seg]); atomicAdd(&out[2], 1ull);
}
}
extern "C" {

OG_API int og_query_stats(const og_query *q, og_stats *out) {
    if (!q || !out) return OG_E_INVAL;
    og_query *mq = const_cast<og_query *>(q);
    if (q->ran && q->stats.page_bytes == 0) {
        CU(cudaSetDevice(q->sh->device));
        Scratch tmp;
        unsigned long long *d_o; int rc = tmp.get(&d_o, 3); if (rc) return rc;
        cudaMemset(d_o, 0, 24);
        if (q->sh->n_segments) k_sum_page_bytes<<<(q->sh->n_segments + 255) / 256, 256>>>(make_dir(q->sh), q->qp, q->qp.tmin, q->qp.tmax, d_o);
        unsigned long long h[3]; CU(cudaMemcpy(h, d_o, 24, cudaMemcpyDeviceToHost));
        mq->stats.page_bytes = h[0]; mq->stats.rows_decoded = h[1]; mq->stats.segments_scanned = h[2];
    }
    *out = q->stats;
    return OG_OK;
}

OG_API int og_query_merge_dense(og_query *q, const og_dense_view *other) {
    if (!q || !other) return OG_E_INVAL;
    if (!q->ran) return OG_E_STATE;
    const QueryP &p = q->qp;
    if (other->n_groups != q->n_groups || other->n_buckets != p.n_buckets || other->n_cols != p.n_calls) { set_error("dense shapes differ"); return OG_E_INVAL; }
    if (other->start != (q->desc.interval ? p.start : 0) || other->interval != (q->desc.interval ? p.interval : 0)) {
        set_error("dense grids differ (start %lld vs %lld, interval %lld vs %lld): create the queries with OG_Q_QUERY_GRID", (long long)other->start,
                  (long long)(q->desc.interval ? p.start : 0), (long long)other->interval, (long long)(q->desc.interval ? p.interval : 0));
        return OG_E_INVAL;
    }
    CU(cudaSetDevice(q->sh->device));
    GroupP mine, oth; memset(&mine, 0, sizeof mine); memset(&oth, 0, sizeof oth);
    mine.n_groups = oth.n_groups = q->n_groups;
    for (uint32_t c = 0; c < p.n_calls; c++) {
        if (other->cols[c].func != p.calls[c].func || other->cols[c].type != p.calls[c].out_type) {
            set_error("dense column %u: func %d type %d, this query's is func %d type %d", c, other->cols[c].func, other->cols[c].type, p.calls[c].func,
                      p.calls[c].out_type);
            return OG_E_INVAL;
        }
        mine.dense[c] = q->dense[c];
        oth.dense[c].val = (uint64_t *)other->cols[c].values; oth.dense[c].ok = other->cols[c].valid; oth.dense[c].tim = other->cols[c].times;
        if ((q->dense[c].tim != nullptr) != (oth.dense[c].tim != nullptr)) { set_error("dense column %u: times presence differs", c); return OG_E_INVAL; }
    }
    size_t total = (size_t)q->n_groups * p.n_buckets;
    k_merge_dense<<<(unsigned)((total + 255) / 256), 256, 0, q->stream>>>(p, mine, oth);
    CU(cudaGetLastError());
    CU(cudaStreamSynchronize(q->stream));
    q->host_ready = false;
    return OG_OK;
}

OG_API int og_query_next(og_query *q, og_record_view *out) {
    if (!q || !out) return OG_E_INVAL;
    if (!q->ran) { set_error("og_query_next before og_query_run"); return OG_E_STATE; }
    if (q->aborted) return OG_E_ABORTED;
    const QueryP &p = q->qp;
    size_t total = (size_t)q->n_groups * p.n_buckets;
    if (!q->host_ready) {
        CU(cudaSetDevice(q->sh->device));
        for (uint32_t c = 0; c < p.n_calls; c++) {
            q->h_val[c].resize(total); q->h_ok[c].resize(total);
            CU(cudaMemcpy(q->h_val[c].data(), q->dense[c].val, total * 8, cudaMemcpyDeviceToHost));
            CU(cudaMemcpy(q->h_ok[c].data(), q->dense[c].ok, total, cudaMemcpyDeviceToHost));
            if (q->dense[c].tim) { q->h_tim[c].resize(total); CU(cudaMemcpy(q->h_tim[c].data(), q->dense[c].tim, total * 8, cudaMemcpyDeviceToHost)); }
        }
        q->host_ready = true; q->next_group = 0; q->next_row = 0;
    }
    int chunk = q->desc.chunk_size > 0 ? q->desc.chunk_size : 1024;
    uint32_t nc = p.n_calls;
    q->rv_val.assign(nc, {}); q->rv_bitmap.assign(nc, {}); q->rv_coltimes.assign(nc, {}); q->rv_times.clear(); q->rv_cols.assign(nc, og_colval_view{});
    while (q->next_group < q->n_groups) {
        uint32_t g = q->next_group;
        std::vector<int32_t> nil(nc, 0);
        int rows = 0;
        uint32_t b = q->next_row;
        uint32_t b_end = (uint32_t)std::min<uint64_t>(p.n_buckets, (uint64_t)b + (uint64_t)chunk);
        for (; b < b_end; b++) {
            const uint32_t bb = q->desc.ascending ? b : p.n_buckets - 1 - b;
            size_t i = (size_t)g * p.n_buckets + bb;
            bool any = false;
            for (uint32_t c = 0; c < nc; c++) any |= q->h_ok[c][i] != 0;
            if (!any) continue;
            int64_t row_time = p.start + (int64_t)bb * p.interval;
            if (q->desc.interval == 0) row_time = 0;
            for (uint32_t c = 0; c < nc; c++) {
                bool ok = q->h_ok[c][i] != 0;
                if ((size_t)(rows >> 3) >= q->rv_bitmap[c].size()) q->rv_bitmap[c].push_back(0);
                if (ok) {
                    q->rv_bitmap[c][rows >> 3] |= (uint8_t)(1 << (rows & 7));
                    if (p.calls[c].out_type == OG_TYPE_BOOL) q->rv_val[c].push_back((uint8_t)(q->h_val[c][i] != 0));
                    else { const uint8_t *pv = (const uint8_t *)&q->h_val[c][i]; q->rv_val[c].insert(q->rv_val[c].end(), pv, pv + 8); }
                } else nil[c]++;
                if (q->dense[c].tim) {
                    if (p.multi) q->rv_coltimes[c].push_back(ok ? q->h_tim[c][i] : 0);
                    else if (ok) row_time = q->h_tim[c][i];
                }
            }
            q->rv_times.push_back(row_time);
            rows++;
        }
        q->next_row = b_end;
        if (q->next_row >= p.n_buckets) { q->next_group++; q->next_row = 0; }
        if (rows == 0) continue;
        for (uint32_t c = 0; c < nc; c++) {
            og_colval_view &v = q->rv_cols[c];
            v.val = q->rv_val[c].data(); v.val_bytes = q->rv_val[c].size(); v.bitmap = q->rv_bitmap[c].data();
            v.times = (p.multi && q->dense[c].tim) ? q->rv_coltimes[c].data() : nullptr;
            v.type = p.calls[c].out_type; v.len = rows; v.nil_count = nil[c]; v.bitmap_offset = 0;
        }
        out->n_cols = nc; out->cols = q->rv_cols.data(); out->times = q->rv_times.data(); out->rows = rows; out->group = g;
        out->sid = q->desc.group_mode == OG_GROUP_PER_SERIES ? q->sh->sids[g] : 0;
        return OG_OK;
    }
    return OG_EOF;
}

}
namespace {
__global__ void k_decode_column(DirP d, uint32_t column, int type, uint32_t seg_begin, uint32_t seg_end, uint8_t *out, uint64_t stride,
                                uint32_t *rows_out, uint8_t *bitmap_out, uint32_t bitmap_stride, int *err) {
    uint32_t seg = seg_begin + blockIdx.x * blockDim.x + threadIdx.x;
    if (seg >= seg_end) return;
    uint8_t *o = out + (size_t)(seg - seg_begin) * stride;
    uint32_t rows = d.seg_rows[seg];
    size_t pi = (size_t)column * d.n_segments + seg;
    if (column == d.n_columns) {
        TimeDesc t;
        int rc = parse_time_page(d.data + d.page_off[pi], d.page_len[pi], t);
        if (rc == D_OK) {
            TimeIter it; it.init(t);
            for (uint32_t i = 0; i < t.rows; i++) ((int64_t *)o)[i] = it.next();
            it.finish(); rc = it.err;
        }
        if (rc != D_OK) report_err(err, rc, seg);
        if (rows_out) rows_out[seg - seg_begin] = rows;
        return;
    }
    uint32_t len = d.page_len[pi];
    uint8_t *bm = bitmap_out ? bitmap_out + (size_t)(seg - seg_begin) * bitmap_stride : nullptr;
    if (len == 0) {
        if (rows_out) rows_out[seg - seg_begin] = 0;
        if (bm) for (uint32_t i = 0; i < (rows + 7) / 8; i++) bm[i] = 0;
        return;
    }
    ColIter it;
    it.init(d.data + d.page_off[pi], len, type, rows);
    int rc = it.err;
    if (rc == D_OK && type == OG_TYPE_STRING) rc = D_UNSUPPORTED;
    if (rc == D_OK) {
        const PageHdr &h = it.h;
        for (uint32_t r = 0, j = 0; r < rows; r++) {
            uint64_t v;
            if (!it.next(v)) continue;
            if (type == OG_TYPE_BOOL) o[j++] = (uint8_t)v; else ((uint64_t *)o)[j++] = v;
        }
        it.finish(); rc = it.err;
        if (rows_out) rows_out[seg - seg_begin] = h.rows - h.nil_count;
        if (bm) {
            for (uint32_t i = 0; i < (rows + 7) / 8; i++) {
                uint8_t v = 0;
                for (uint32_t k = 0; k < 8 && i * 8 + k < rows; k++) v |= (uint8_t)(hdr_row_valid(h, i * 8 + k) ? 1 : 0) << k;
                bm[i] = v;
            }
        }
    }
    if (rc != D_OK) report_err(err, rc, seg);
}
}
extern "C" {

OG_API int og_decode_column_device(og_shard *s, uint32_t column, uint32_t seg_begin, uint32_t seg_end, void *d_values,
                                   uint64_t value_stride_bytes, uint32_t *d_rows_out) {
    if (!s || !d_values || column > s->n_columns || seg_begin > seg_end || seg_end > s->n_segments) { set_error("bad argument"); return OG_E_INVAL; }
    CU(cudaSetDevice(s->device));
    if (seg_begin == seg_end) return OG_OK;
    int *d_err; int rc = dalloc(&d_err, 2); if (rc) return rc;
    cudaMemset(d_err, 0, 8);
    int type = column == s->n_columns ? OG_TYPE_INT : s->col_types[column];
    uint32_t n = seg_end - seg_begin;
    k_decode_column<<<(n + 127) / 128, 128>>>(make_dir(s), column, type, seg_begin, seg_end, (uint8_t *)d_values, value_stride_bytes, d_rows_out, nullptr, 0, d_err);
    int err[2]; cudaError_t e = cudaMemcpy(err, d_err, 8, cudaMemcpyDeviceToHost); dev_free(d_err);
    if (e != cudaSuccess) return cuda_fail(e, "k_decode_column", __FILE__, __LINE__);
    if (err[0]) { set_error("segment %d failed to decode (device code %d)", err[1], err[0]); return map_dev_err(err[0]); }
    return OG_OK;
}

__global__ void k_reverse_segment(uint8_t *vals, uint32_t elem_bytes, uint32_t n_vals, uint8_t *bitmap, uint32_t rows) {
    for (uint32_t i = threadIdx.x; i < n_vals / 2; i += blockDim.x) {
        const uint32_t j = n_vals - 1 - i;
        if (elem_bytes == 8) { uint64_t *v = (uint64_t *)vals; const uint64_t a = v[i]; v[i] = v[j]; v[j] = a; }
        else { const uint8_t a = vals[i]; vals[i] = vals[j]; vals[j] = a; }
    }
    if (!bitmap) return;
    __syncthreads();
    __shared__ uint8_t sbm[8192];
    const uint32_t nb = (rows + 7) / 8;
    for (uint32_t i = threadIdx.x; i < nb; i += blockDim.x) sbm[i] = bitmap[i];
    __syncthreads();
    for (uint32_t i = threadIdx.x; i < nb; i += blockDim.x) {
        uint8_t o = 0;
        for (uint32_t k = 0; k < 8 && i * 8 + k < rows; k++) { const uint32_t src = rows - 1 - (i * 8 + k); o |= (uint8_t)((sbm[src >> 3] >> (src & 7)) & 1) << k; }
        bitmap[i] = o;
    }
}
}
static int decode_segment_impl(og_shard *s, uint32_t segment, uint32_t flags, og_record_view *out);
extern "C" {
OG_API int og_decode_segment(og_shard *s, uint32_t segment, og_record_view *out) { return decode_segment_impl(s, segment, 0, out); }
OG_API int og_decode_segment_ex(og_shard *s, uint32_t segment, uint32_t flags, og_record_view *out) { return decode_segment_impl(s, segment, flags, out); }
}
static int decode_segment_impl(og_shard *s, uint32_t segment, uint32_t flags, og_record_view *out) {
    if (!s || !out || segment >= s->n_segments) { set_error("bad argument"); return OG_E_INVAL; }
    CU(cudaSetDevice(s->device));
    uint32_t R = std::max<uint32_t>(1, s->max_seg_rows);
    size_t ncol1 = (size_t)s->n_columns + 1;
    size_t val_stride = (size_t)R * 8, bm_stride = (((size_t)R + 7) / 8 + 7) & ~(size_t)7;
    size_t need = ncol1 * (val_stride + bm_stride + 16);
    if (s->d_seg_buf_bytes < need || s->h_seg_buf_bytes < need) {
        dev_free(s->d_seg_buf); s->d_seg_buf = nullptr; s->d_seg_buf_bytes = 0;
        if (s->h_seg_buf) cudaFreeHost(s->h_seg_buf);
        s->h_seg_buf = nullptr; s->h_seg_buf_bytes = 0;
        CU(dev_malloc(&s->d_seg_buf, need)); s->d_seg_buf_bytes = need;
        CU(cudaMallocHost(&s->h_seg_buf, need)); s->h_seg_buf_bytes = need;
    }
    uint8_t *dv = (uint8_t *)s->d_seg_buf, *dbm = dv + ncol1 * val_stride;
    uint32_t *drows = (uint32_t *)(dbm + ncol1 * bm_stride);
    int *d_err; int rc = dalloc(&d_err, 2); if (rc) return rc;
    cudaMemset(d_err, 0, 8);
    DirP dir = make_dir(s);
    for (uint32_t c = 0; c <= s->n_columns; c++) {
        int type = c == s->n_columns ? OG_TYPE_INT : s->col_types[c];
        k_decode_column<<<1, 32>>>(dir, c, type, segment, segment + 1, dv + c * val_stride, val_stride, drows + c, dbm + c * bm_stride, (uint32_t)bm_stride, d_err);
    }
    int err[2]; cudaError_t e = cudaMemcpy(err, d_err, 8, cudaMemcpyDeviceToHost); dev_free(d_err);
    if (e != cudaSuccess) return cuda_fail(e, "k_decode_column", __FILE__, __LINE__);
    if (err[0]) { set_error("segment %d failed to decode (device code %d)", err[1], err[0]); return map_dev_err(err[0]); }
    if (flags & OG_DECODE_DESCENDING) {
        if (R > 65536) { set_error("descending materialisation supports segments of up to 65536 rows"); return OG_E_UNSUPPORTED; }
        uint32_t hr[65];
        CU(cudaMemcpy(hr, drows, (ncol1) * 4, cudaMemcpyDeviceToHost));
        const uint32_t rows_seg = hr[s->n_columns];
        for (uint32_t c = 0; c <= s->n_columns; c++) {
            const bool is_time = c == s->n_columns;
            const uint32_t eb = (!is_time && s->col_types[c] == OG_TYPE_BOOL) ? 1 : 8;
            k_reverse_segment<<<1, 256>>>(dv + c * val_stride, eb, is_time ? rows_seg : hr[c], is_time ? nullptr : dbm + c * bm_stride, rows_seg);
        }
        CU(cudaGetLastError());
    }
    CU(cudaMemcpy(s->h_seg_buf, s->d_seg_buf, need, cudaMemcpyDeviceToHost));
    uint8_t *hv = (uint8_t *)s->h_seg_buf, *hbm = hv + ncol1 * val_stride;
    uint32_t *hrows = (uint32_t *)(hbm + ncol1 * bm_stride);
    uint32_t rows = hrows[s->n_columns];
    s->seg_views.assign(s->n_columns, og_colval_view{});
    for (uint32_t c = 0; c < s->n_columns; c++) {
        og_colval_view &v = s->seg_views[c];
        uint32_t nv = hrows[c];
        v.val = hv + c * val_stride; v.val_bytes = (uint64_t)nv * (s->col_types[c] == OG_TYPE_BOOL ? 1 : 8);
        v.bitmap = hbm + c * bm_stride; v.times = nullptr; v.type = s->col_types[c]; v.len = (int32_t)rows; v.nil_count = (int32_t)(rows - nv); v.bitmap_offset = 0;
    }
    out->n_cols = s->n_columns; out->cols = s->seg_views.data(); out->times = (const int64_t *)(hv + s->n_columns * val_stride); out->rows = (int32_t)rows; out->group = 0;
    uint32_t sr = (uint32_t)(std::upper_bound(s->h_series_seg_begin.begin(), s->h_series_seg_begin.end(), segment) - s->h_series_seg_begin.begin()) - 1;
    out->sid = s->sids[sr];
    return OG_OK;
}
```

opengemini_b200/csrc/fused_il.cuh:

```cuda
#pragma once
#include "agg_kernels.cuh"

namespace ogpu {

__device__ __forceinline__ uint32_t smem_u32(const void *p) { return (uint32_t)__cvta_generic_to_shared(p); }
__device__ __forceinline__ uint32_t opaque(uint32_t x) { asm volatile("mov.u32 %0, %0;" : "+r"(x)); return x; }
template <int OFF> __device__ __forceinline__ uint32_t lds32o(uint32_t a) { uint32_t v; asm volatile("ld.shared.u32 %0, [%1+%2];" : "=r"(v) : "r"(a), "n"(OFF)); return v; }
__device__ __forceinline__ void mbar_init(uint32_t bar, uint32_t count) { asm volatile("mbarrier.init.shared::cta.b64 [%0], %1;" ::"r"(bar), "r"(count) : "memory"); }
__device__ __forceinline__ void mbar_init_fence() { asm volatile("fence.mbarrier_init.release.cluster;\nfence.proxy.async.shared::cta;" ::: "memory"); }
__device__ __forceinline__ void mbar_expect_tx(uint32_t bar, uint32_t bytes) { asm volatile("mbarrier.arrive.expect_tx.shared::cta.b64 _, [%0], %1;" ::"r"(bar), "r"(bytes) : "memory"); }
__device__ __forceinline__ void bulk_g2s(uint32_t dst, const void *src, uint32_t bytes, uint32_t bar) {
    asm volatile("cp.async.bulk.shared::cluster.global.mbarrier::complete_tx::bytes [%0], [%1], %2, [%3];" ::"r"(dst), "l"(src), "r"(bytes), "r"(bar) : "memory");
}
__device__ __forceinline__ bool mbar_wait(uint32_t bar, uint32_t parity) {
#pragma unroll 1
    for (uint32_t i = 0; i < (1u << 16); i++) {
        uint32_t ok;
        asm volatile("{\n.reg .pred p;\nmbarrier.try_wait.parity.shared::cta.b64 p, [%1], %2;\nselp.u32 %0, 1, 0, p;\n}" : "=r"(ok) : "r"(bar), "r"(parity) : "memory");
        if (ok) return true;
    }
    return false;
}

enum { FM_COUNT = 1, FM_SUM = 2, FM_MIN = 4, FM_MAX = 8, FM_FIRST = 16, FM_LAST = 32 };
enum { SEG_GENERAL = 0, SEG_FAST = 1, SEG_PACKED = 2 };

#ifndef OG_FAST_THREADS
#define OG_FAST_THREADS 128
#endif
#ifndef OG_FAST_MAXREG
#define OG_FAST_MAXREG 80
#endif
#ifndef OG_IL_NW
#define OG_IL_NW 64u
#endif
#ifndef OG_IL_B
#define OG_IL_B 16u
#endif
#ifndef OG_IL_K
#define OG_IL_K 10u
#endif
#ifndef OG_IL_UNROLL
#define OG_IL_UNROLL 2
#endif
#define OG_IL_NB (OG_IL_NW / OG_IL_B)
#define OG_IL_ROWS (OG_IL_NW + 2u)
#define OG_IL_PAD_WORDS 6u
#define OG_IL_HDR 7u
#define OG_IL_RAW_HDR 6u
#define OG_IL_NONE 0xffffffffu
#define OG_IL_PACKED 0x8000u
#define OG_IL_LOOKBITS (77u * OG_IL_K + 29u + 13u + 64u + 64u)
static_assert(OG_IL_K >= 2, "packed lanes: K*64 + 63 + 128 <= OG_IL_LOOKBITS needs K >= 2");
static_assert(OG_IL_NW % OG_IL_B == 0 && (OG_IL_NW & (OG_IL_NW - 1)) == 0, "ring geometry");
static_assert(OG_IL_NW - OG_IL_B > (OG_IL_LOOKBITS + 31u) / 32u + 2u, "ring too small for the round length: the slowest lane could not proceed");

struct IlP {
    const uint32_t *words;
    const uint64_t *grp_off;
    const uint32_t *grp_rows;
    const uint32_t *grp_col;
    const uint32_t *lane_seg;
    const uint32_t *lane_rows;
    const uint16_t *lane_win;
    const uint32_t *lane_series;
    const int64_t *lane_t0;
    const uint64_t *lane_dt;
};

__device__ __forceinline__ uint64_t udiv_est(uint64_t a, uint64_t b, double inv_b) {
    const double qd = __ull2double_rn(a) * inv_b;
    if ((a >> 63) || !(qd < 1125899906842624.0)) return a / b;
    uint64_t q = (uint64_t)qd;
    uint64_t r = a - q * b;
    if ((int64_t)r < 0) { do { q--; r += b; } while ((int64_t)r < 0); }
    else while (r >= b) { q++; r -= b; }
    return q;
}

__device__ __forceinline__ uint64_t fetch64(uint32_t col, uint32_t p) {
    uint32_t a = col + ((p << 2) & ((OG_IL_NW - 1) << 7));
    uint32_t a0 = lds32o<0>(a), a1 = lds32o<128>(a), a2 = lds32o<256>(a);
    uint32_t hi = __funnelshift_l(a1, a0, p), lo = __funnelshift_l(a2, a1, p);
    return ((uint64_t)hi << 32) | lo;
}

__device__ __forceinline__ Part fold32(int func, int type, bool multi, Part p, bool with_time) {
    constexpr uint32_t FULL = 0xffffffffu;
    if (func == OG_AGG_COUNT) { p.v = __reduce_add_sync(FULL, p.ok ? (uint32_t)p.v : 0u); p.ok = p.v != 0; return p; }
    if (type == OG_TYPE_FLOAT && func == OG_AGG_SUM) {
        double s = p.ok ? u2d(p.v) : 0.0;
#pragma unroll
        for (int o = 16; o; o >>= 1) s += __shfl_xor_sync(FULL, s, o);
        p.ok = __any_sync(FULL, p.ok != 0); p.v = d2u(s); return p;
    }
    if (type == OG_TYPE_FLOAT && !with_time && (func == OG_AGG_MIN || func == OG_AGG_MAX)) {
        double v = u2d(p.v); uint32_t ok = p.ok;
#pragma unroll
        for (int o = 16; o; o >>= 1) {
            const double ov = __shfl_xor_sync(FULL, v, o); const uint32_t ook = __shfl_xor_sync(FULL, ok, o);
            const bool keep = ok && (func == OG_AGG_MIN ? v <= ov : v >= ov);
            if (ook && !keep) v = ov;
            ok |= ook;
        }
        p.v = d2u(v); p.ok = ok; return p;
    }
    return warp_fold(func, type, multi, p, with_time);
}

#define OG_IL_WCAP 24u
__host__ __device__ inline uint32_t il_acc_bytes(uint32_t n_calls, bool times) { return OG_IL_WCAP * n_calls * (times ? 17u : 9u) + 8u & ~7u; }

template <int FM, bool TIMES, bool FOLD>
__global__ void __maxnreg__(OG_FAST_MAXREG) k_fused_il(QueryP q, ChunkP ch, IlP il, uint32_t grp_begin, uint32_t grp_end) {
    constexpr uint32_t NW = OG_IL_NW, B = OG_IL_B, NB = OG_IL_NB, K = OG_IL_K;
    constexpr uint32_t FULL = 0xffffffffu;
    constexpr uint32_t WPB = OG_FAST_THREADS / 32;
    constexpr int UNR = OG_IL_UNROLL;
    __shared__ __align__(128) uint32_t s_win[WPB * OG_IL_ROWS * 32];
    __shared__ __align__(8) uint64_t s_bar[WPB * NB];
    extern __shared__ __align__(8) uint8_t s_acc[];

#ifdef OG_IL_STATS
    const long long st_clk0 = clock64();
    long long st_wait = 0;
#endif
    const uint32_t lane = threadIdx.x & 31;
    const uint32_t wid = __reduce_max_sync(FULL, threadIdx.x >> 5);
    const uint32_t grp = grp_begin + blockIdx.x * WPB + wid;
    if (grp >= grp_end) return;
    const uint32_t rows_w = __reduce_max_sync(FULL, il.grp_rows[grp]);
    if (rows_w == 0) return;
    const size_t slot = (size_t)grp * 32 + lane;
    const uint32_t seg = il.lane_seg[slot];
    bool active = seg != OG_IL_NONE && seg >= ch.seg_begin && seg < ch.seg_end;
    if (!__any_sync(FULL, active)) return;
    const size_t e = 2 * (size_t)(seg - ch.seg_begin);

    uint32_t rows = 0, series = 0, r_lo = 0, r_hi = 0, lwin = 0;
    int64_t t0 = 0, dt = 1; uint64_t dtu = 1; double inv_dt = 1.0;
    const double inv_iv = 1.0 / __ull2double_rn((uint64_t)q.interval);
    if (active) {
        rows = il.lane_rows[slot]; lwin = il.lane_win[slot]; series = il.lane_series[slot];
        t0 = il.lane_t0[slot]; dtu = il.lane_dt[slot]; dt = (int64_t)dtu;
        inv_dt = 1.0 / __ull2double_rn(dtu);
        r_lo = 0; r_hi = rows - 1;
        if (t0 < q.tmin) { uint64_t k = udiv_est((uint64_t)(q.tmin - t0) + dtu - 1, dtu, inv_dt); r_lo = k > rows ? rows : (uint32_t)k; }
        { int64_t t_last = t0 + (int64_t)(rows - 1) * dt; if (t_last > q.tmax) { if (q.tmax < t0) r_lo = rows; else r_hi = (uint32_t)udiv_est((uint64_t)(q.tmax - t0), dtu, inv_dt); } }
        const uint64_t span = (uint64_t)q.n_buckets * (uint64_t)q.interval;
        const bool outside = r_lo <= r_hi && r_lo < rows &&
                             ((uint64_t)(t0 + (int64_t)r_lo * dt - q.start) >= span || (uint64_t)(t0 + (int64_t)r_hi * dt - q.start) >= span);
        if (outside) report_err(ch.err, D_CORRUPT, seg);
        if (r_lo > r_hi || r_lo >= rows || outside) { *(uint2 *)(ch.edge_bucket + e) = make_uint2(OG_NO_BUCKET, OG_NO_BUCKET); active = false; }
    }
    if (!__any_sync(FULL, active)) return;

    const uint32_t win = smem_u32(s_win) + wid * (OG_IL_ROWS * 128);
    const uint32_t col = opaque(win + lane * 4);
    const uint32_t bar0 = smem_u32(s_bar) + wid * (NB * 8);
    if (lane == 0) {
#pragma unroll
        for (uint32_t i = 0; i < NB; i++) mbar_init(bar0 + i * 8, 1);
        mbar_init_fence();
    }
    __syncwarp();
    const uint32_t total_b = rows_w / B;
    uint64_t goff = il.grp_off[grp];
    goff = ((uint64_t)__reduce_max_sync(FULL, (uint32_t)(goff >> 32)) << 32) | __reduce_max_sync(FULL, (uint32_t)goff);
    const uint32_t *gsrc = il.words + goff;
    uint32_t issued_b = 0, ready_b = 0;
    uint32_t hung = 0;
    uint64_t pol;
    asm("createpolicy.fractional.L2::evict_first.b64 %0, 1.0;" : "=l"(pol));
    auto issue = [&](uint32_t k_any) {
        const uint32_t k = __reduce_max_sync(FULL, k_any);
        const uint32_t s = k % NB, dst = win + s * (B * 128), bar = bar0 + s * 8;
        const uint32_t *src = gsrc + (size_t)k * (B * 32);
        if (s == 0)
            asm volatile("{\n.reg .pred p;\nelect.sync _|p, 0xffffffff;\n@p mbarrier.arrive.expect_tx.shared::cta.b64 _, [%0], %1;\n"
                         "@p cp.async.bulk.shared::cluster.global.mbarrier::complete_tx::bytes.L2::cache_hint [%2], [%3], %4, [%0], %6;\n"
                         "@p cp.async.bulk.shared::cluster.global.mbarrier::complete_tx::bytes.L2::cache_hint [%5], [%3], 256, [%0], %6;\n}"
                         ::"r"(bar), "r"(B * 128 + 256u), "r"(dst), "l"(src), "r"(B * 128), "r"(win + NW * 128), "l"(pol) : "memory");
        else
            asm volatile("{\n.reg .pred p;\nelect.sync _|p, 0xffffffff;\n@p mbarrier.arrive.expect_tx.shared::cta.b64 _, [%0], %1;\n"
                         "@p cp.async.bulk.shared::cluster.global.mbarrier::complete_tx::bytes.L2::cache_hint [%2], [%3], %1, [%0], %4;\n}"
                         ::"r"(bar), "r"(B * 128), "r"(dst), "l"(src), "l"(pol) : "memory");
    };
    {
        const uint32_t first = total_b < NB ? total_b : NB;
        for (uint32_t k = 0; k < first; k++) issue(k);
        issued_b = first;
    }

    uint32_t cur_b = 0, rb = 0xffffffffu, step_q = 0; uint64_t rem = 0, step_r = 0;
    if (active) {
        const int64_t t_lo = t0 + (int64_t)r_lo * dt;
        cur_b = (uint32_t)udiv_est((uint64_t)(t_lo - q.start), (uint64_t)q.interval, inv_iv);
        const uint64_t ivl = (uint64_t)q.interval;
        const uint64_t sq64 = udiv_est(ivl, dtu, inv_dt);
        step_q = sq64 > 0xffffffffull ? 0xffffffffu : (uint32_t)sq64;
        step_r = ivl - sq64 * dtu;
        uint64_t D = (uint64_t)(q.start + (int64_t)(cur_b + 1) * q.interval - t0) + dtu - 1;
        uint64_t qq = udiv_est(D, dtu, inv_dt); rem = D - qq * dtu; rb = qq > 0xffffffffull ? 0xffffffffu : (uint32_t)qq;
    }

    bool uni = false; uint32_t b0 = 0, b_end = 0;
    uint64_t *acc_v = nullptr; int64_t *acc_t = nullptr; uint8_t *acc_k = nullptr;
    if (FOLD) {
        const int leader = __ffs(__ballot_sync(FULL, active)) - 1;
        const int64_t t0L = __shfl_sync(FULL, t0, leader); const uint64_t dtL = __shfl_sync(FULL, dtu, leader);
        const uint32_t loL = __shfl_sync(FULL, r_lo, leader), hiL = __shfl_sync(FULL, r_hi, leader);
        b0 = __shfl_sync(FULL, cur_b, leader);
        const bool same = t0 == t0L && dtu == dtL && r_lo == loL && r_hi == hiL;
        const uint32_t b_last = active ? (uint32_t)udiv_est((uint64_t)(t0 + (int64_t)r_hi * dt - q.start), (uint64_t)q.interval, inv_iv) : b0;
        uni = __all_sync(FULL, !active || (same && b_last - b0 < OG_IL_WCAP));
        if (uni) {
            b_end = __reduce_max_sync(FULL, active ? b_last : 0u);
            const uint32_t nacc = OG_IL_WCAP * q.n_calls;
            uint8_t *base = s_acc + (size_t)wid * il_acc_bytes(q.n_calls, TIMES);
            acc_v = (uint64_t *)base; acc_t = (int64_t *)(base + (size_t)nacc * 8); acc_k = base + (size_t)nacc * (TIMES ? 16 : 8);
            for (uint32_t i = lane; i < nacc; i += 32) acc_k[i] = 0;
            __syncwarp();
        }
    }
    const uint32_t gcol = FOLD ? il.grp_col[grp] - ch.gc_col0 : 0;
    const bool fold_edges = FOLD && uni && b_end > b0;

    double sum = 0.0, mn = 0.0, mx = 0.0; uint64_t fi = 0, lastv = 0;
    uint32_t n_mn = 0, n_mx = 0;
    uint32_t w_row0 = r_lo;
    bool head_done = false; uint32_t head_b = OG_NO_BUCKET;
    uint32_t stop = 0, n_ev = 0;
    auto part_of = [&](int func, uint32_t cnt) -> Part {
        Part pp; pp.ok = cnt != 0; pp.v = 0; pp.t = 0;
        switch (func) {
        case OG_AGG_COUNT: pp.v = cnt; break;
        case OG_AGG_SUM: if (FM & FM_SUM) pp.v = d2u(sum); break;
        case OG_AGG_MIN: if (FM & FM_MIN) { pp.v = d2u(mn); if (TIMES) pp.t = t0 + (int64_t)(stop - n_mn) * dt; } break;
        case OG_AGG_MAX: if (FM & FM_MAX) { pp.v = d2u(mx); if (TIMES) pp.t = t0 + (int64_t)(stop - n_mx) * dt; } break;
        case OG_AGG_FIRST: if (FM & FM_FIRST) { pp.v = fi; pp.t = t0 + (int64_t)w_row0 * dt; } break;
        default: if (FM & FM_LAST) { pp.v = lastv; pp.t = t0 + (int64_t)(stop - 1) * dt; } break;
        }
        return pp;
    };
    auto kind_of = [&]() -> int { return !head_done ? 0 : stop > r_hi ? 1 : 2; };
    auto flush_lane = [&](int kind) {
        const uint32_t cnt = stop - w_row0;
#pragma unroll 1
        for (uint32_t c = 0; c < q.n_calls; c++) {
            const Part pp = part_of(q.calls[c].func, cnt);
            if (kind == 2) { if (pp.ok) store_cell(ch, (int)c, series, cur_b, pp); }
            else store_part(ch.edges[c], e + kind, pp);
        }
        if (kind == 0) { head_done = true; head_b = cur_b; }
    };
    auto flush_fold = [&](bool ev) {
        uint32_t pend = __ballot_sync(FULL, ev);
#pragma unroll 1
        while (pend) {
            const int leader = __ffs(pend) - 1;
            const uint32_t bL = __shfl_sync(FULL, cur_b, leader);
            const bool mine = ev && cur_b == bL;
            const uint32_t cnt = mine ? stop - w_row0 : 0;
            const uint32_t w = bL - b0;
#pragma unroll 1
            for (uint32_t c = 0; c < q.n_calls; c++) {
                const int func = q.calls[c].func, ftype = func == OG_AGG_COUNT ? OG_TYPE_INT : q.calls[c].type;
                const bool wt = func >= OG_AGG_MIN && !(q.multi && func <= OG_AGG_MAX);
                Part pp = fold32(func, ftype, q.multi != 0, part_of(func, cnt), wt);
                if ((int)lane == leader && pp.ok) {
                    const uint32_t i = c * OG_IL_WCAP + w;
                    Part a; a.ok = acc_k[i]; a.v = a.ok ? acc_v[i] : 0; a.t = (TIMES && a.ok) ? acc_t[i] : 0;
                    group_update(func, ftype, q.multi != 0, a, pp);
                    acc_v[i] = a.v; acc_k[i] = 1; if (TIMES) acc_t[i] = a.t;
                }
            }
            pend &= ~__ballot_sync(FULL, mine);
        }
        __syncwarp();
    };

    uint32_t qp = 0, sr = 0, kfast = 0, CM = 0, CE = 0, m = 64, tr = 0, bad = 0; uint64_t MASK = 0;
    bool done = !active;
    uint64_t val = 0;

#ifdef OG_IL_STATS
    long long st_w0 = clock64();
#endif
    if (issued_b && !mbar_wait(bar0, 0)) hung = 1; else ready_b = issued_b ? 1 : 0;
#ifdef OG_IL_STATS
    st_wait += clock64() - st_w0;
#endif
    if (active && !hung) {
        val = fetch64(col, 0); qp = 64;
        if (lwin & OG_IL_PACKED) {
            const uint32_t lead = (lwin >> 8) & 63u, mw = lwin & 127u;
            qp = 64 - lead; kfast = mw;
            MASK = mw ? (~0ull >> (64 - mw)) << (64 - lead - mw) : 0ull;
        } else { CM = 0; CE = 1; }
    }

    bool skipping = r_lo > 0;
    stop = skipping ? r_lo : (rb < r_hi + 1 ? rb : r_hi + 1);
    n_ev = stop;
    if (!skipping) { fi = val; mn = mx = u2d(val); n_mn = n_mx = n_ev; }
    if (done) n_ev = 0xffffffffu;

    auto retire = [&]() { done = true; n_ev = 0xffffffffu; CM = 0; CE = 0; MASK = 0; kfast = 0; };
    auto advance = [&]() {
        bool fin = false;
        if (skipping) { skipping = false; sum = 0.0; }
        else {
            fin = stop > r_hi;
            sum = 0.0;
            if (!fin) while (stop >= rb) {
                cur_b++;
                rem += step_r; uint32_t adv = step_q;
                if (rem >= dtu) { rem -= dtu; adv++; }
                rb = (rb > 0xffffffffu - adv) ? 0xffffffffu : rb + adv;
            }
        }
        if (fin) retire();
        else {
            w_row0 = stop;
            uint32_t nstop = rb < r_hi + 1 ? rb : r_hi + 1;
            n_ev = nstop - stop; stop = nstop;
            fi = val; mn = mx = u2d(val); n_mn = n_mx = n_ev;
        }
    };
    auto slow_record = [&]() {
        uint32_t p = qp + sr;
        const uint64_t x = fetch64(col, p);
        const uint32_t ctrl = (uint32_t)(x >> 62);
        if (ctrl < 2) { qp += 1; return; }
        if (ctrl == 3) {
            const uint32_t lm = (uint32_t)(x >> 51) & 0x7ff;
            uint32_t lead = lm >> 6; m = lm & 0x3f;
            if (m == 0) { m = 64; tr = 0; lead = 0; }
            else { if (lead + m > 64) { if (!done) bad = 1; lead = 0; m = 64; } tr = 64 - lead - m; }
            p += 13;
            const bool slowwin = lead < 2;
            sr = slowwin ? 0 : lead - 2;
            CM = slowwin ? 0u : 3u << (30 - sr); CE = slowwin ? 1u : 2u << (30 - sr);
            kfast = 2 + m;
            MASK = (m == 64 ? ~0ull : ((1ull << m) - 1)) << tr;
        } else p += 2;
        const uint64_t y = fetch64(col, p);
        const uint64_t sig = m == 64 ? y : (y >> (64 - m));
        p += m;
        val ^= sig << tr;
        qp = p - sr;
    };
    auto accumulate = [&](uint32_t k_in_run) {
        if (FM & FM_SUM) sum = sum + u2d(val);
        if (FM & FM_MIN) { if (mn > u2d(val)) { mn = u2d(val); if (TIMES) n_mn = n_ev - k_in_run; } }
        if (FM & FM_MAX) { if (mx < u2d(val)) { mx = u2d(val); if (TIMES) n_mx = n_ev - k_in_run; } }
        if (FM & FM_LAST) lastv = val;
    };
    auto record = [&](uint32_t k_in_run) {
        accumulate(k_in_run);
        const uint64_t x = fetch64(col, qp);
        const bool slow = (((uint32_t)(x >> 32) & CM) ^ CE) != 0;
        if (slow) slow_record();
        else { val ^= x & MASK; qp += kfast; }
    };
    auto record2 = [&](uint32_t k_in_run) {
        const uint64_t x0 = fetch64(col, qp), x1 = fetch64(col, qp + kfast);
        accumulate(k_in_run);
#ifdef OG_IL_REC2B
        uint64_t x1b = x1;
        if ((((uint32_t)(x0 >> 32) & CM) ^ CE) != 0) { slow_record(); x1b = fetch64(col, qp); }
        else { val ^= x0 & MASK; qp += kfast; }
        accumulate(k_in_run + 1);
        if ((((uint32_t)(x1b >> 32) & CM) ^ CE) != 0) slow_record();
        else { val ^= x1b & MASK; qp += kfast; }
#else
        if ((((uint32_t)(x0 >> 32) & CM) ^ CE) != 0) { slow_record(); record(k_in_run + 1); return; }
        val ^= x0 & MASK; qp += kfast;
        accumulate(k_in_run + 1);
        if ((((uint32_t)(x1 >> 32) & CM) ^ CE) != 0) slow_record();
        else { val ^= x1 & MASK; qp += kfast; }
#endif
    };

    uint32_t rounds_left = hung ? 0u : 40u * (__reduce_max_sync(FULL, rows) / K + 8u);
#ifdef OG_IL_STATS
    uint32_t st_common = 0, st_rare = 0, st_sit = 0, st_notgo = 0;
    const long long st_pro = clock64() - st_clk0;
#endif
    for (;;) {
        const uint32_t qmin = __reduce_min_sync(FULL, done ? 0xffffffffu : qp);
        if (qmin == 0xffffffffu) break;
        const uint32_t f = qmin < 32 ? 0u : (qmin - 32) >> 5;
#pragma unroll 1
        while (issued_b < total_b && (issued_b + 1) * B <= f + NW) { issue(issued_b); issued_b++; }
        const uint32_t qmax = __reduce_max_sync(FULL, done ? 0u : qp);
        uint32_t need_max = ((qmax + OG_IL_LOOKBITS) >> 5) + 1; if (need_max > rows_w) need_max = rows_w;
        uint32_t want_b = (need_max + B - 1) / B; if (want_b > issued_b) want_b = issued_b;
#ifdef OG_IL_STATS
        st_w0 = clock64();
#endif
#pragma unroll 1
        while (ready_b < want_b) { if (!mbar_wait(bar0 + (ready_b % NB) * 8, (ready_b / NB) & 1)) { hung = 1; break; } ready_b++; }
#ifdef OG_IL_STATS
        st_wait += clock64() - st_w0;
#endif
        if (hung) break;
        uint32_t need = ((qp + OG_IL_LOOKBITS) >> 5) + 1; if (need > rows_w) need = rows_w;
        bool go = done || need <= ready_b * B;
        uint32_t run = __reduce_min_sync(FULL, go ? n_ev : 0u);
        if (run >= K) {
            static_assert(K % 2 == 0, "records are decoded in pairs");
#pragma unroll UNR
            for (uint32_t k = 0; k < K; k += 2) record2(k);
            n_ev -= K;
#ifdef OG_IL_STATS
            st_common++;
#endif
            continue;
        }
#ifdef OG_IL_STATS
        st_rare++;
#endif
        if (rounds_left-- == 0) { hung = 2; break; }
        const bool all_go = __all_sync(FULL, go);
#ifdef OG_IL_STATS
        if (!all_go) { st_notgo++; st_sit += __popc(__ballot_sync(FULL, !go)); }
#endif
        uint32_t left = K;
        for (;;) {
            run = __reduce_min_sync(FULL, go ? n_ev : 0xffffffffu);
            if (run > left) run = left;
            if (all_go) {
#pragma unroll 1
                for (uint32_t k = 0; k < run; k++) record(k);
            } else {
#pragma unroll 1
                for (uint32_t k = 0; k < run; k++) if (go) record(k);
            }
            if (go) n_ev -= run;
            left -= run;
            if (left == 0) break;
            const bool ev = go && !done && n_ev == 0;
            if (FOLD && uni) {
                const bool fl = ev && !skipping;
                const int kind = kind_of();
                const bool to_acc = fl && (kind == 2 || fold_edges);
                if (fl && !to_acc) flush_lane(kind);
                if (__any_sync(FULL, to_acc)) flush_fold(to_acc);
                if (to_acc && kind == 0) head_done = true;
            } else if (ev && !skipping) flush_lane(kind_of());
            if (ev) advance();
            if (__all_sync(FULL, ev || done)) break;
        }
    }
    if (active && (qp >> 5) >= rows_w) bad = 1;
#ifdef OG_IL_STATS
    const long long st_e0 = clock64();
    if (lane == 0) { atomicAdd((unsigned *)&ch.err[4], st_common); atomicAdd((unsigned *)&ch.err[5], st_rare); atomicAdd((unsigned *)&ch.err[6], st_notgo); atomicAdd((unsigned *)&ch.err[7], st_sit); }
#endif
    while (ready_b < issued_b && hung != 1) { if (!mbar_wait(bar0 + (ready_b % NB) * 8, (ready_b / NB) & 1)) hung = 1; ready_b++; }
    if (hung && lane == 0) report_err(ch.err, D_WATCHDOG, (grp << 2) | hung);
    if (FOLD && uni) {
        __syncwarp();
        const uint32_t w_tail = fold_edges ? b_end - b0 : OG_IL_WCAP;
        for (uint32_t i = lane; i < OG_IL_WCAP * q.n_calls; i += 32) {
            if (!acc_k[i]) continue;
            const uint32_t c = i / OG_IL_WCAP, w = i % OG_IL_WCAP;
            Part a; a.ok = 1; a.v = acc_v[i]; a.t = TIMES ? acc_t[i] : 0;
            store_part(ch.gcells[c], (size_t)(b0 + w) * ch.gc_cols + (w == w_tail ? ch.gc_tail0 + gcol : gcol), a);
        }
    }
    if (FOLD && __any_sync(FULL, active && head_b != OG_NO_BUCKET) && lane == 0) ch.flags[1] = 1;
    if (active) {
        if (bad) report_err(ch.err, D_CORRUPT, seg);
        *(uint2 *)(ch.edge_bucket + e) = make_uint2(head_b, (head_b == OG_NO_BUCKET || cur_b == head_b) ? OG_NO_BUCKET : cur_b);
    }
#ifdef OG_IL_STATS
    if (lane == 0) {
        atomicAdd((unsigned long long *)(ch.err + 8), (unsigned long long)st_wait);
        const long long st_end = clock64();
        atomicAdd((unsigned long long *)(ch.err + 10), (unsigned long long)(st_end - st_clk0));
        atomicAdd((unsigned long long *)(ch.err + 12), (unsigned long long)st_pro);
        atomicAdd((unsigned long long *)(ch.err + 14), (unsigned long long)(st_end - st_e0));
    }
#endif
}

}
```

Before: 500.6 billion.

## Make IL decode kernel persistent with atomic group claiming and cross-group prefetch

Converts k_fused_il from one warp per group into a persistent kernel sized to occupancy. Each warp claims groups through an atomic counter and starts the bulk copies for the next group's words into the same smem ring while finishing the current one. It also prefetches the next group's lane metadata into L2 and uses a smaller copy batch size (OG_IL_CB). The merge kernel skips edge columns when no head edges were flagged. This adds per-group atomics and more complex ring bookkeeping, which brings hang and ordering risk, and adds host-side occupancy queries on every launch.

```diff
diff --git a/opengemini_b200/csrc/agg_kernels.cuh b/opengemini_b200/csrc/agg_kernels.cuh
--- a/opengemini_b200/csrc/agg_kernels.cuh
+++ b/opengemini_b200/csrc/agg_kernels.cuh
@@ -472,7 +472,8 @@
     const Tri g = ch.gcells[c];
     Part acc = part_empty();
     const size_t row = (size_t)b * ch.gc_cols;
-    for (uint32_t col = lane; col < ch.gc_cols; col += 32) {
+    const uint32_t n_cols = ch.gc_edge0 && !ch.flags[1] ? ch.gc_edge0 : ch.gc_cols;
+    for (uint32_t col = lane; col < n_cols; col += 32) {
         if (!g.ok[row + col]) continue;
         Part p; p.ok = 1; p.v = g.val[row + col]; p.t = wt ? g.tim[row + col] : 0;
         group_update(func, ftype, multi, acc, p);
diff --git a/opengemini_b200/csrc/api.cu b/opengemini_b200/csrc/api.cu
--- a/opengemini_b200/csrc/api.cu
+++ b/opengemini_b200/csrc/api.cu
@@ -442,9 +442,16 @@
 }
 template <int FM, bool TIMES> void launch_fast_t(bool fold, const IlP &il, uint32_t g0, uint32_t g1, const QueryP &p, const ChunkP &ch, cudaStream_t st) {
     constexpr uint32_t WPB = OG_FAST_THREADS / 32;
-    dim3 grid((g1 - g0 + WPB - 1) / WPB), block(OG_FAST_THREADS);
-    if (fold) k_fused_il<FM, TIMES, true><<<grid, block, WPB * il_acc_bytes(p.n_calls, TIMES), st>>>(p, ch, il, g0, g1);
-    else k_fused_il<FM, TIMES, false><<<grid, block, 0, st>>>(p, ch, il, g0, g1);
+    const size_t smem = fold ? WPB * il_acc_bytes(p.n_calls, TIMES) : 0;
+    auto kern = fold ? k_fused_il<FM, TIMES, true> : k_fused_il<FM, TIMES, false>;
+    int dev = 0, n_sm = 0, per_sm = 0;
+    cudaGetDevice(&dev);
+    cudaDeviceGetAttribute(&n_sm, cudaDevAttrMultiProcessorCount, dev);
+    cudaOccupancyMaxActiveBlocksPerMultiprocessor(&per_sm, kern, OG_FAST_THREADS, smem);
+    size_t blocks = std::min<size_t>((g1 - g0 + WPB - 1) / WPB, (size_t)std::max(1, per_sm) * std::max(1, n_sm));
+    if (const char *ov = getenv("OGPU_IL_BLOCKS")) { long v = atol(ov); if (v > 0) blocks = std::min<size_t>(blocks, (size_t)v); }
+    cudaMemsetAsync(il.claim, 0, sizeof(uint32_t), st);
+    kern<<<(unsigned)blocks, OG_FAST_THREADS, smem, st>>>(p, ch, il, g0, g1);
 }
 void launch_fast(int fm, bool times, bool fold, const IlP &il, uint32_t g0, uint32_t g1, const QueryP &p, const ChunkP &ch, cudaStream_t st) {
     if (g1 <= g0) return;
@@ -728,6 +735,7 @@
     if (pl->fast) {
         pl->il.words = ic->words; pl->il.grp_off = ic->grp_off; pl->il.grp_rows = ic->grp_rows; pl->il.grp_col = ic->grp_col;
         pl->il.lane_seg = ic->lane_seg; pl->il.lane_rows = ic->lane_rows; pl->il.lane_win = ic->lane_win; pl->il.lane_series = ic->lane_series; pl->il.lane_t0 = ic->lane_t0; pl->il.lane_dt = ic->lane_dt;
+        if ((rc = q->bufs.get(&pl->il.claim, 1))) return rc;
         pl->fm = 0; pl->times = false;
         for (uint32_t c = 0; c < p.n_calls; c++) {
             pl->fm |= 1 << (p.calls[c].func - 1);
diff --git a/opengemini_b200/csrc/fused_il.cuh b/opengemini_b200/csrc/fused_il.cuh
--- a/opengemini_b200/csrc/fused_il.cuh
+++ b/opengemini_b200/csrc/fused_il.cuh
@@ -43,7 +43,10 @@
 #ifndef OG_IL_UNROLL
 #define OG_IL_UNROLL 2
 #endif
-#define OG_IL_NB (OG_IL_NW / OG_IL_B)
+#ifndef OG_IL_CB
+#define OG_IL_CB 8u
+#endif
+#define OG_IL_NB (OG_IL_NW / OG_IL_CB)
 #define OG_IL_ROWS (OG_IL_NW + 2u)
 #define OG_IL_PAD_WORDS 6u
 #define OG_IL_HDR 7u
@@ -52,8 +55,8 @@
 #define OG_IL_PACKED 0x8000u
 #define OG_IL_LOOKBITS (77u * OG_IL_K + 29u + 13u + 64u + 64u)
 static_assert(OG_IL_K >= 2, "packed lanes: K*64 + 63 + 128 <= OG_IL_LOOKBITS needs K >= 2");
-static_assert(OG_IL_NW % OG_IL_B == 0 && (OG_IL_NW & (OG_IL_NW - 1)) == 0, "ring geometry");
-static_assert(OG_IL_NW - OG_IL_B > (OG_IL_LOOKBITS + 31u) / 32u + 2u, "ring too small for the round length: the slowest lane could not proceed");
+static_assert(OG_IL_NW % OG_IL_CB == 0 && OG_IL_B % OG_IL_CB == 0 && (OG_IL_NW & (OG_IL_NW - 1)) == 0, "ring geometry");
+static_assert(OG_IL_NW - OG_IL_CB > (OG_IL_LOOKBITS + 31u) / 32u + 2u, "ring too small for the round length: the slowest lane could not proceed");
 
 struct IlP {
     const uint32_t *words;
@@ -66,6 +69,7 @@
     const uint32_t *lane_series;
     const int64_t *lane_t0;
     const uint64_t *lane_dt;
+    uint32_t *claim;
 };
 
 __device__ __forceinline__ uint64_t udiv_est(uint64_t a, uint64_t b, double inv_b) {
@@ -113,7 +117,7 @@
 
 template <int FM, bool TIMES, bool FOLD>
 __global__ void __maxnreg__(OG_FAST_MAXREG) k_fused_il(QueryP q, ChunkP ch, IlP il, uint32_t grp_begin, uint32_t grp_end) {
-    constexpr uint32_t NW = OG_IL_NW, B = OG_IL_B, NB = OG_IL_NB, K = OG_IL_K;
+    constexpr uint32_t NW = OG_IL_NW, B = OG_IL_CB, NB = OG_IL_NB, K = OG_IL_K;
     constexpr uint32_t FULL = 0xffffffffu;
     constexpr uint32_t WPB = OG_FAST_THREADS / 32;
     constexpr int UNR = OG_IL_UNROLL;
@@ -122,38 +126,12 @@
     extern __shared__ __align__(8) uint8_t s_acc[];
 
 #ifdef OG_IL_STATS
-    const long long st_clk0 = clock64();
-    long long st_wait = 0;
+    const long long st_k0 = clock64();
+    long long st_wait = 0, st_pro = 0, st_epi = 0;
+    uint32_t st_common = 0, st_rare = 0, st_sit = 0, st_notgo = 0;
 #endif
     const uint32_t lane = threadIdx.x & 31;
     const uint32_t wid = __reduce_max_sync(FULL, threadIdx.x >> 5);
-    const uint32_t grp = grp_begin + blockIdx.x * WPB + wid;
-    if (grp >= grp_end) return;
-    const uint32_t rows_w = __reduce_max_sync(FULL, il.grp_rows[grp]);
-    if (rows_w == 0) return;
-    const size_t slot = (size_t)grp * 32 + lane;
-    const uint32_t seg = il.lane_seg[slot];
-    bool active = seg != OG_IL_NONE && seg >= ch.seg_begin && seg < ch.seg_end;
-    if (!__any_sync(FULL, active)) return;
-    const size_t e = 2 * (size_t)(seg - ch.seg_begin);
-
-    uint32_t rows = 0, series = 0, r_lo = 0, r_hi = 0, lwin = 0;
-    int64_t t0 = 0, dt = 1; uint64_t dtu = 1; double inv_dt = 1.0;
-    const double inv_iv = 1.0 / __ull2double_rn((uint64_t)q.interval);
-    if (active) {
-        rows = il.lane_rows[slot]; lwin = il.lane_win[slot]; series = il.lane_series[slot];
-        t0 = il.lane_t0[slot]; dtu = il.lane_dt[slot]; dt = (int64_t)dtu;
-        inv_dt = 1.0 / __ull2double_rn(dtu);
-        r_lo = 0; r_hi = rows - 1;
-        if (t0 < q.tmin) { uint64_t k = udiv_est((uint64_t)(q.tmin - t0) + dtu - 1, dtu, inv_dt); r_lo = k > rows ? rows : (uint32_t)k; }
-        { int64_t t_last = t0 + (int64_t)(rows - 1) * dt; if (t_last > q.tmax) { if (q.tmax < t0) r_lo = rows; else r_hi = (uint32_t)udiv_est((uint64_t)(q.tmax - t0), dtu, inv_dt); } }
-        const uint64_t span = (uint64_t)q.n_buckets * (uint64_t)q.interval;
-        const bool outside = r_lo <= r_hi && r_lo < rows &&
-                             ((uint64_t)(t0 + (int64_t)r_lo * dt - q.start) >= span || (uint64_t)(t0 + (int64_t)r_hi * dt - q.start) >= span);
-        if (outside) report_err(ch.err, D_CORRUPT, seg);
-        if (r_lo > r_hi || r_lo >= rows || outside) { *(uint2 *)(ch.edge_bucket + e) = make_uint2(OG_NO_BUCKET, OG_NO_BUCKET); active = false; }
-    }
-    if (!__any_sync(FULL, active)) return;
 
     const uint32_t win = smem_u32(s_win) + wid * (OG_IL_ROWS * 128);
     const uint32_t col = opaque(win + lane * 4);
@@ -164,327 +142,405 @@
         mbar_init_fence();
     }
     __syncwarp();
-    const uint32_t total_b = rows_w / B;
-    uint64_t goff = il.grp_off[grp];
-    goff = ((uint64_t)__reduce_max_sync(FULL, (uint32_t)(goff >> 32)) << 32) | __reduce_max_sync(FULL, (uint32_t)goff);
-    const uint32_t *gsrc = il.words + goff;
-    uint32_t issued_b = 0, ready_b = 0;
-    uint32_t hung = 0;
     uint64_t pol;
     asm("createpolicy.fractional.L2::evict_first.b64 %0, 1.0;" : "=l"(pol));
-    auto issue = [&](uint32_t k_any) {
-        const uint32_t k = __reduce_max_sync(FULL, k_any);
-        const uint32_t s = k % NB, dst = win + s * (B * 128), bar = bar0 + s * 8;
-        const uint32_t *src = gsrc + (size_t)k * (B * 32);
-        if (s == 0)
-            asm volatile("{\n.reg .pred p;\nelect.sync _|p, 0xffffffff;\n@p mbarrier.arrive.expect_tx.shared::cta.b64 _, [%0], %1;\n"
-                         "@p cp.async.bulk.shared::cluster.global.mbarrier::complete_tx::bytes.L2::cache_hint [%2], [%3], %4, [%0], %6;\n"
-                         "@p cp.async.bulk.shared::cluster.global.mbarrier::complete_tx::bytes.L2::cache_hint [%5], [%3], 256, [%0], %6;\n}"
-                         ::"r"(bar), "r"(B * 128 + 256u), "r"(dst), "l"(src), "r"(B * 128), "r"(win + NW * 128), "l"(pol) : "memory");
-        else
-            asm volatile("{\n.reg .pred p;\nelect.sync _|p, 0xffffffff;\n@p mbarrier.arrive.expect_tx.shared::cta.b64 _, [%0], %1;\n"
-                         "@p cp.async.bulk.shared::cluster.global.mbarrier::complete_tx::bytes.L2::cache_hint [%2], [%3], %1, [%0], %4;\n}"
-                         ::"r"(bar), "r"(B * 128), "r"(dst), "l"(src), "l"(pol) : "memory");
+    auto claim = [&]() -> uint32_t {
+        uint32_t c = 0;
+        if (lane == 0) c = atomicAdd(il.claim, 1u);
+        c = __reduce_max_sync(FULL, c);
+        return c < grp_end - grp_begin ? grp_begin + c : grp_end;
     };
-    {
-        const uint32_t first = total_b < NB ? total_b : NB;
-        for (uint32_t k = 0; k < first; k++) issue(k);
-        issued_b = first;
+    auto group_src = [&](uint32_t g, const uint32_t *&src, uint32_t &nbatch) {
+        nbatch = 0; src = il.words;
+        if (g >= grp_end) return;
+        nbatch = __reduce_max_sync(FULL, il.grp_rows[g]) / B;
+        const uint64_t goff = il.grp_off[g];
+        src = il.words + (((uint64_t)__reduce_max_sync(FULL, (uint32_t)(goff >> 32)) << 32) | __reduce_max_sync(FULL, (uint32_t)goff));
+    };
+    auto prefetch_meta = [&](uint32_t g) {
+        if (g >= grp_end) return;
+        const size_t s0 = (size_t)g * 32;
+        const void *p = lane == 0 ? (const void *)(il.lane_seg + s0) : lane == 1 ? (const void *)(il.lane_rows + s0)
+                      : lane == 2 ? (const void *)(il.lane_win + s0) : lane == 3 ? (const void *)(il.lane_series + s0)
+                      : lane < 6 ? (const void *)(il.lane_t0 + s0 + (lane - 4) * 16) : lane < 8 ? (const void *)(il.lane_dt + s0 + (lane - 6) * 16)
+                      : lane == 8 ? (const void *)(il.grp_col + g) : nullptr;
+        if (p) asm volatile("prefetch.global.L2 [%0];" ::"l"(p) : "memory");
+    };
+    uint32_t grp = claim();
+    const uint32_t *gsrc; uint32_t total_b;
+    group_src(grp, gsrc, total_b);
+    uint32_t sb0 = 0, issued = 0, ready = 0;
+    uint32_t hung = 0;
+    while (grp < grp_end && !hung) {
+        uint32_t nxt = grp_end, ntotal_b = 0; const uint32_t *nsrc = il.words;
+        bool have_next = false;
+        auto next_group = [&]() {
+            if (have_next) return;
+            nxt = claim();
+            prefetch_meta(nxt);
+            group_src(nxt, nsrc, ntotal_b);
+            have_next = true;
+        };
+        auto issue = [&](uint32_t k_any) {
+            const uint32_t k = __reduce_max_sync(FULL, k_any), kr = k - sb0;
+            const uint32_t s = k % NB, dst = win + s * (B * 128), bar = bar0 + s * 8;
+            const uint32_t *src = kr < total_b ? gsrc + (size_t)kr * (B * 32) : nsrc + (size_t)(kr - total_b) * (B * 32);
+            if (s == 0)
+                asm volatile("{\n.reg .pred p;\nelect.sync _|p, 0xffffffff;\n@p mbarrier.arrive.expect_tx.shared::cta.b64 _, [%0], %1;\n"
+                             "@p cp.async.bulk.shared::cluster.global.mbarrier::complete_tx::bytes.L2::cache_hint [%2], [%3], %4, [%0], %6;\n"
+                             "@p cp.async.bulk.shared::cluster.global.mbarrier::complete_tx::bytes.L2::cache_hint [%5], [%3], 256, [%0], %6;\n}"
+                             ::"r"(bar), "r"(B * 128 + 256u), "r"(dst), "l"(src), "r"(B * 128), "r"(win + NW * 128), "l"(pol) : "memory");
+            else
+                asm volatile("{\n.reg .pred p;\nelect.sync _|p, 0xffffffff;\n@p mbarrier.arrive.expect_tx.shared::cta.b64 _, [%0], %1;\n"
+                             "@p cp.async.bulk.shared::cluster.global.mbarrier::complete_tx::bytes.L2::cache_hint [%2], [%3], %1, [%0], %4;\n}"
+                             ::"r"(bar), "r"(B * 128), "r"(dst), "l"(src), "l"(pol) : "memory");
+        };
+        auto refill = [&](uint32_t f) {
+#pragma unroll 1
+            while (issued - sb0 < total_b + ntotal_b && (issued - sb0 + 1) * B <= f + NW) { issue(issued); issued++; }
+        };
+        auto wait_to = [&](uint32_t k_end) {
+#pragma unroll 1
+            while (ready < k_end) { if (!mbar_wait(bar0 + (ready % NB) * 8, (ready / NB) & 1)) { hung = 1; break; } ready++; }
+        };
+        auto run_group = [&]() {
+#ifdef OG_IL_STATS
+            const long long st_clk0 = clock64();
+#endif
+            const uint32_t rows_w = total_b * B;
+            if (rows_w == 0) return;
+            refill(0);
+            next_group();
+            const size_t slot = (size_t)grp * 32 + lane;
+            const uint32_t seg = il.lane_seg[slot];
+            bool active = seg != OG_IL_NONE && seg >= ch.seg_begin && seg < ch.seg_end;
+            if (!__any_sync(FULL, active)) return;
+            const size_t e = 2 * (size_t)(seg - ch.seg_begin);
+
+            uint32_t rows = 0, series = 0, r_lo = 0, r_hi = 0, lwin = 0;
+            int64_t t0 = 0, dt = 1; uint64_t dtu = 1; double inv_dt = 1.0;
+            const double inv_iv = 1.0 / __ull2double_rn((uint64_t)q.interval);
+            if (active) {
+                rows = il.lane_rows[slot]; lwin = il.lane_win[slot]; series = il.lane_series[slot];
+                t0 = il.lane_t0[slot]; dtu = il.lane_dt[slot]; dt = (int64_t)dtu;
+                inv_dt = 1.0 / __ull2double_rn(dtu);
+                r_lo = 0; r_hi = rows - 1;
+                if (t0 < q.tmin) { uint64_t k = udiv_est((uint64_t)(q.tmin - t0) + dtu - 1, dtu, inv_dt); r_lo = k > rows ? rows : (uint32_t)k; }
+                { int64_t t_last = t0 + (int64_t)(rows - 1) * dt; if (t_last > q.tmax) { if (q.tmax < t0) r_lo = rows; else r_hi = (uint32_t)udiv_est((uint64_t)(q.tmax - t0), dtu, inv_dt); } }
+                const uint64_t span = (uint64_t)q.n_buckets * (uint64_t)q.interval;
+                const bool outside = r_lo <= r_hi && r_lo < rows &&
+                                     ((uint64_t)(t0 + (int64_t)r_lo * dt - q.start) >= span || (uint64_t)(t0 + (int64_t)r_hi * dt - q.start) >= span);
+                if (outside) report_err(ch.err, D_CORRUPT, seg);
+                if (r_lo > r_hi || r_lo >= rows || outside) { *(uint2 *)(ch.edge_bucket + e) = make_uint2(OG_NO_BUCKET, OG_NO_BUCKET); active = false; }
+            }
+            if (!__any_sync(FULL, active)) return;
+
+            const uint32_t rb32 = (sb0 % NB) * (B * 32);
+
+            uint32_t cur_b = 0, rb = 0xffffffffu, step_q = 0; uint64_t rem = 0, step_r = 0;
+            if (active) {
+                const int64_t t_lo = t0 + (int64_t)r_lo * dt;
+                cur_b = (uint32_t)udiv_est((uint64_t)(t_lo - q.start), (uint64_t)q.interval, inv_iv);
+                const uint64_t ivl = (uint64_t)q.interval;
+                const uint64_t sq64 = udiv_est(ivl, dtu, inv_dt);
+                step_q = sq64 > 0xffffffffull ? 0xffffffffu : (uint32_t)sq64;
+                step_r = ivl - sq64 * dtu;
+                uint64_t D = (uint64_t)(q.start + (int64_t)(cur_b + 1) * q.interval - t0) + dtu - 1;
+                uint64_t qq = udiv_est(D, dtu, inv_dt); rem = D - qq * dtu; rb = qq > 0xffffffffull ? 0xffffffffu : (uint32_t)qq;
+            }
+
+            bool uni = false; uint32_t b0 = 0, b_end = 0;
+            uint64_t *acc_v = nullptr; int64_t *acc_t = nullptr; uint8_t *acc_k = nullptr;
+            if (FOLD) {
+                const int leader = __ffs(__ballot_sync(FULL, active)) - 1;
+                const int64_t t0L = __shfl_sync(FULL, t0, leader); const uint64_t dtL = __shfl_sync(FULL, dtu, leader);
+                const uint32_t loL = __shfl_sync(FULL, r_lo, leader), hiL = __shfl_sync(FULL, r_hi, leader);
+                b0 = __shfl_sync(FULL, cur_b, leader);
+                const bool same = t0 == t0L && dtu == dtL && r_lo == loL && r_hi == hiL;
+                const uint32_t b_last = active ? (uint32_t)udiv_est((uint64_t)(t0 + (int64_t)r_hi * dt - q.start), (uint64_t)q.interval, inv_iv) : b0;
+                uni = __all_sync(FULL, !active || (same && b_last - b0 < OG_IL_WCAP));
+                if (uni) {
+                    b_end = __reduce_max_sync(FULL, active ? b_last : 0u);
+                    const uint32_t nacc = OG_IL_WCAP * q.n_calls;
+                    uint8_t *base = s_acc + (size_t)wid * il_acc_bytes(q.n_calls, TIMES);
+                    acc_v = (uint64_t *)base; acc_t = (int64_t *)(base + (size_t)nacc * 8); acc_k = base + (size_t)nacc * (TIMES ? 16 : 8);
+                    for (uint32_t i = lane; i < nacc; i += 32) acc_k[i] = 0;
+                    __syncwarp();
+                }
+            }
+            const uint32_t gcol = FOLD ? il.grp_col[grp] - ch.gc_col0 : 0;
+            const bool fold_edges = FOLD && uni && b_end > b0;
+
+            double sum = 0.0, mn = 0.0, mx = 0.0; uint64_t fi = 0, lastv = 0;
+            uint32_t n_mn = 0, n_mx = 0;
+            uint32_t w_row0 = r_lo;
+            bool head_done = false; uint32_t head_b = OG_NO_BUCKET;
+            uint32_t stop = 0, n_ev = 0;
+            auto part_of = [&](int func, uint32_t cnt) -> Part {
+                Part pp; pp.ok = cnt != 0; pp.v = 0; pp.t = 0;
+                switch (func) {
+                case OG_AGG_COUNT: pp.v = cnt; break;
+                case OG_AGG_SUM: if (FM & FM_SUM) pp.v = d2u(sum); break;
+                case OG_AGG_MIN: if (FM & FM_MIN) { pp.v = d2u(mn); if (TIMES) pp.t = t0 + (int64_t)(stop - n_mn) * dt; } break;
+                case OG_AGG_MAX: if (FM & FM_MAX) { pp.v = d2u(mx); if (TIMES) pp.t = t0 + (int64_t)(stop - n_mx) * dt; } break;
+                case OG_AGG_FIRST: if (FM & FM_FIRST) { pp.v = fi; pp.t = t0 + (int64_t)w_row0 * dt; } break;
+                default: if (FM & FM_LAST) { pp.v = lastv; pp.t = t0 + (int64_t)(stop - 1) * dt; } break;
+                }
+                return pp;
+            };
+            auto kind_of = [&]() -> int { return !head_done ? 0 : stop > r_hi ? 1 : 2; };
+            auto flush_lane = [&](int kind) {
+                const uint32_t cnt = stop - w_row0;
+#pragma unroll 1
+                for (uint32_t c = 0; c < q.n_calls; c++) {
+                    const Part pp = part_of(q.calls[c].func, cnt);
+                    if (kind == 2) { if (pp.ok) store_cell(ch, (int)c, series, cur_b, pp); }
+                    else store_part(ch.edges[c], e + kind, pp);
+                }
+                if (kind == 0) { head_done = true; head_b = cur_b; }
+            };
+            auto flush_fold = [&](bool ev) {
+                uint32_t pend = __ballot_sync(FULL, ev);
+#pragma unroll 1
+                while (pend) {
+                    const int leader = __ffs(pend) - 1;
+                    const uint32_t bL = __shfl_sync(FULL, cur_b, leader);
+                    const bool mine = ev && cur_b == bL;
+                    const uint32_t cnt = mine ? stop - w_row0 : 0;
+                    const uint32_t w = bL - b0;
+#pragma unroll 1
+                    for (uint32_t c = 0; c < q.n_calls; c++) {
+                        const int func = q.calls[c].func, ftype = func == OG_AGG_COUNT ? OG_TYPE_INT : q.calls[c].type;
+                        const bool wt = func >= OG_AGG_MIN && !(q.multi && func <= OG_AGG_MAX);
+                        Part pp = fold32(func, ftype, q.multi != 0, part_of(func, cnt), wt);
+                        if ((int)lane == leader && pp.ok) {
+                            const uint32_t i = c * OG_IL_WCAP + w;
+                            Part a; a.ok = acc_k[i]; a.v = a.ok ? acc_v[i] : 0; a.t = (TIMES && a.ok) ? acc_t[i] : 0;
+                            group_update(func, ftype, q.multi != 0, a, pp);
+                            acc_v[i] = a.v; acc_k[i] = 1; if (TIMES) acc_t[i] = a.t;
+                        }
+                    }
+                    pend &= ~__ballot_sync(FULL, mine);
+                }
+                __syncwarp();
+            };
+
+            uint32_t qp = 0, sr = 0, kfast = 0, CM = 0, CE = 0, m = 64, tr = 0, bad = 0; uint64_t MASK = 0;
+            bool done = !active;
+            uint64_t val = 0;
+
+#ifdef OG_IL_STATS
+            long long st_w0 = clock64();
+#endif
+            wait_to(sb0 + 1);
+#ifdef OG_IL_STATS
+            st_wait += clock64() - st_w0;
+#endif
+            if (active && !hung) {
+                val = fetch64(col, rb32); qp = rb32 + 64;
+                if (lwin & OG_IL_PACKED) {
+                    const uint32_t lead = (lwin >> 8) & 63u, mw = lwin & 127u;
+                    qp = rb32 + 64 - lead; kfast = mw;
+                    MASK = mw ? (~0ull >> (64 - mw)) << (64 - lead - mw) : 0ull;
+                } else { CM = 0; CE = 1; }
+            }
+
+            bool skipping = r_lo > 0;
+            stop = skipping ? r_lo : (rb < r_hi + 1 ? rb : r_hi + 1);
+            n_ev = stop;
+            if (!skipping) { fi = val; mn = mx = u2d(val); n_mn = n_mx = n_ev; }
+            if (done) n_ev = 0xffffffffu;
+
+            auto retire = [&]() { done = true; n_ev = 0xffffffffu; CM = 0; CE = 0; MASK = 0; kfast = 0; };
+            auto advance = [&]() {
+                bool fin = false;
+                if (skipping) { skipping = false; sum = 0.0; }
+                else {
+                    fin = stop > r_hi;
+                    sum = 0.0;
+                    if (!fin) while (stop >= rb) {
+                        cur_b++;
+                        rem += step_r; uint32_t adv = step_q;
+                        if (rem >= dtu) { rem -= dtu; adv++; }
+                        rb = (rb > 0xffffffffu - adv) ? 0xffffffffu : rb + adv;
+                    }
+                }
+                if (fin) retire();
+                else {
+                    w_row0 = stop;
+                    uint32_t nstop = rb < r_hi + 1 ? rb : r_hi + 1;
+                    n_ev = nstop - stop; stop = nstop;
+                    fi = val; mn = mx = u2d(val); n_mn = n_mx = n_ev;
+                }
+            };
+            auto slow_record = [&]() {
+                uint32_t p = qp + sr;
+                const uint64_t x = fetch64(col, p);
+                const uint32_t ctrl = (uint32_t)(x >> 62);
+                if (ctrl < 2) { qp += 1; return; }
+                if (ctrl == 3) {
+                    const uint32_t lm = (uint32_t)(x >> 51) & 0x7ff;
+                    uint32_t lead = lm >> 6; m = lm & 0x3f;
+                    if (m == 0) { m = 64; tr = 0; lead = 0; }
+                    else { if (lead + m > 64) { if (!done) bad = 1; lead = 0; m = 64; } tr = 64 - lead - m; }
+                    p += 13;
+                    const bool slowwin = lead < 2;
+                    sr = slowwin ? 0 : lead - 2;
+                    CM = slowwin ? 0u : 3u << (30 - sr); CE = slowwin ? 1u : 2u << (30 - sr);
+                    kfast = 2 + m;
+                    MASK = (m == 64 ? ~0ull : ((1ull << m) - 1)) << tr;
+                } else p += 2;
+                const uint64_t y = fetch64(col, p);
+                const uint64_t sig = m == 64 ? y : (y >> (64 - m));
+                p += m;
+                val ^= sig << tr;
+                qp = p - sr;
+            };
+            auto accumulate = [&](uint32_t k_in_run) {
+                if (FM & FM_SUM) sum = sum + u2d(val);
+                if (FM & FM_MIN) { if (mn > u2d(val)) { mn = u2d(val); if (TIMES) n_mn = n_ev - k_in_run; } }
+                if (FM & FM_MAX) { if (mx < u2d(val)) { mx = u2d(val); if (TIMES) n_mx = n_ev - k_in_run; } }
+                if (FM & FM_LAST) lastv = val;
+            };
+            auto record = [&](uint32_t k_in_run) {
+                accumulate(k_in_run);
+                const uint64_t x = fetch64(col, qp);
+                const bool slow = (((uint32_t)(x >> 32) & CM) ^ CE) != 0;
+                if (slow) slow_record();
+                else { val ^= x & MASK; qp += kfast; }
+            };
+            auto record2 = [&](uint32_t k_in_run) {
+                const uint64_t x0 = fetch64(col, qp), x1 = fetch64(col, qp + kfast);
+                accumulate(k_in_run);
+#ifdef OG_IL_REC2B
+                uint64_t x1b = x1;
+                if ((((uint32_t)(x0 >> 32) & CM) ^ CE) != 0) { slow_record(); x1b = fetch64(col, qp); }
+                else { val ^= x0 & MASK; qp += kfast; }
+                accumulate(k_in_run + 1);
+                if ((((uint32_t)(x1b >> 32) & CM) ^ CE) != 0) slow_record();
+                else { val ^= x1b & MASK; qp += kfast; }
+#else
+                if ((((uint32_t)(x0 >> 32) & CM) ^ CE) != 0) { slow_record(); record(k_in_run + 1); return; }
+                val ^= x0 & MASK; qp += kfast;
+                accumulate(k_in_run + 1);
+                if ((((uint32_t)(x1 >> 32) & CM) ^ CE) != 0) slow_record();
+                else { val ^= x1 & MASK; qp += kfast; }
+#endif
+            };
+
+            uint32_t rounds_left = hung ? 0u : 40u * (__reduce_max_sync(FULL, rows) / K + 8u);
+#ifdef OG_IL_STATS
+            st_pro += clock64() - st_clk0;
+#endif
+            while (!hung) {
+                const uint32_t qmin = __reduce_min_sync(FULL, done ? 0xffffffffu : qp);
+                if (qmin == 0xffffffffu) break;
+                const uint32_t qlo = qmin - rb32;
+                refill(qlo < 32 ? 0u : (qlo - 32) >> 5);
+                const uint32_t qmax = __reduce_max_sync(FULL, done ? 0u : qp) - rb32;
+                uint32_t need_max = ((qmax + OG_IL_LOOKBITS) >> 5) + 1; if (need_max > rows_w) need_max = rows_w;
+                uint32_t want_b = (need_max + B - 1) / B; if (want_b > issued - sb0) want_b = issued - sb0;
+#ifdef OG_IL_STATS
+                st_w0 = clock64();
+#endif
+                wait_to(sb0 + want_b);
+#ifdef OG_IL_STATS
+                st_wait += clock64() - st_w0;
+#endif
+                if (hung) break;
+                uint32_t need = ((qp - rb32 + OG_IL_LOOKBITS) >> 5) + 1; if (need > rows_w) need = rows_w;
+                bool go = done || need <= (ready - sb0) * B;
+                uint32_t run = __reduce_min_sync(FULL, go ? n_ev : 0u);
+                if (run >= K) {
+                    static_assert(K % 2 == 0, "records are decoded in pairs");
+#pragma unroll UNR
+                    for (uint32_t k = 0; k < K; k += 2) record2(k);
+                    n_ev -= K;
+#ifdef OG_IL_STATS
+                    st_common++;
+#endif
+                    continue;
+                }
+#ifdef OG_IL_STATS
+                st_rare++;
+#endif
+                if (rounds_left-- == 0) { hung = 2; break; }
+                const bool all_go = __all_sync(FULL, go);
+#ifdef OG_IL_STATS
+                if (!all_go) { st_notgo++; st_sit += __popc(__ballot_sync(FULL, !go)); }
+#endif
+                uint32_t left = K;
+                for (;;) {
+                    run = __reduce_min_sync(FULL, go ? n_ev : 0xffffffffu);
+                    if (run > left) run = left;
+                    if (all_go) {
+#pragma unroll 1
+                        for (uint32_t k = 0; k < run; k++) record(k);
+                    } else {
+#pragma unroll 1
+                        for (uint32_t k = 0; k < run; k++) if (go) record(k);
+                    }
+                    if (go) n_ev -= run;
+                    left -= run;
+                    if (left == 0) break;
+                    const bool ev = go && !done && n_ev == 0;
+                    if (FOLD && uni) {
+                        const bool fl = ev && !skipping;
+                        const int kind = kind_of();
+                        const bool to_acc = fl && (kind == 2 || fold_edges);
+                        if (fl && !to_acc) flush_lane(kind);
+                        if (__any_sync(FULL, to_acc)) flush_fold(to_acc);
+                        if (to_acc && kind == 0) head_done = true;
+                    } else if (ev && !skipping) flush_lane(kind_of());
+                    if (ev) advance();
+                    if (__all_sync(FULL, ev || done)) break;
+                }
+            }
+            if (active && ((qp - rb32) >> 5) >= rows_w) bad = 1;
+#ifdef OG_IL_STATS
+            const long long st_e0 = clock64();
+#endif
+            if (hung != 1) wait_to(min(issued, sb0 + total_b));
+            if (FOLD && uni) {
+                __syncwarp();
+                const uint32_t w_tail = fold_edges ? b_end - b0 : OG_IL_WCAP;
+                for (uint32_t i = lane; i < OG_IL_WCAP * q.n_calls; i += 32) {
+                    if (!acc_k[i]) continue;
+                    const uint32_t c = i / OG_IL_WCAP, w = i % OG_IL_WCAP;
+                    Part a; a.ok = 1; a.v = acc_v[i]; a.t = TIMES ? acc_t[i] : 0;
+                    store_part(ch.gcells[c], (size_t)(b0 + w) * ch.gc_cols + (w == w_tail ? ch.gc_tail0 + gcol : gcol), a);
+                }
+            }
+            if (FOLD && __any_sync(FULL, active && head_b != OG_NO_BUCKET) && lane == 0) ch.flags[1] = 1;
+            if (active) {
+                if (bad) report_err(ch.err, D_CORRUPT, seg);
+                *(uint2 *)(ch.edge_bucket + e) = make_uint2(head_b, (head_b == OG_NO_BUCKET || cur_b == head_b) ? OG_NO_BUCKET : cur_b);
+            }
+#ifdef OG_IL_STATS
+            const long long st_end = clock64();
+            st_epi += st_end - st_e0;
+#endif
+        };
+        run_group();
+        next_group();
+        if (hung != 1) wait_to(min(issued, sb0 + total_b));
+        if (hung) {
+            if (lane == 0) report_err(ch.err, D_WATCHDOG, (grp << 2) | hung);
+            if (hung == 2) wait_to(issued);
+            break;
+        }
+        sb0 = min(issued, sb0 + total_b);
+        grp = nxt; gsrc = nsrc; total_b = ntotal_b;
     }
-
-    uint32_t cur_b = 0, rb = 0xffffffffu, step_q = 0; uint64_t rem = 0, step_r = 0;
-    if (active) {
-        const int64_t t_lo = t0 + (int64_t)r_lo * dt;
-        cur_b = (uint32_t)udiv_est((uint64_t)(t_lo - q.start), (uint64_t)q.interval, inv_iv);
-        const uint64_t ivl = (uint64_t)q.interval;
-        const uint64_t sq64 = udiv_est(ivl, dtu, inv_dt);
-        step_q = sq64 > 0xffffffffull ? 0xffffffffu : (uint32_t)sq64;
-        step_r = ivl - sq64 * dtu;
-        uint64_t D = (uint64_t)(q.start + (int64_t)(cur_b + 1) * q.interval - t0) + dtu - 1;
-        uint64_t qq = udiv_est(D, dtu, inv_dt); rem = D - qq * dtu; rb = qq > 0xffffffffull ? 0xffffffffu : (uint32_t)qq;
+#ifdef OG_IL_STATS
+    if (lane == 0) {
+        atomicAdd((unsigned *)&ch.err[4], st_common); atomicAdd((unsigned *)&ch.err[5], st_rare); atomicAdd((unsigned *)&ch.err[6], st_notgo); atomicAdd((unsigned *)&ch.err[7], st_sit);
+        atomicAdd((unsigned long long *)(ch.err + 8), (unsigned long long)st_wait);
+        atomicAdd((unsigned long long *)(ch.err + 10), (unsigned long long)(clock64() - st_k0));
+        atomicAdd((unsigned long long *)(ch.err + 12), (unsigned long long)st_pro);
+        atomicAdd((unsigned long long *)(ch.err + 14), (unsigned long long)st_epi);
     }
-
-    bool uni = false; uint32_t b0 = 0, b_end = 0;
-    uint64_t *acc_v = nullptr; int64_t *acc_t = nullptr; uint8_t *acc_k = nullptr;
-    if (FOLD) {
-        const int leader = __ffs(__ballot_sync(FULL, active)) - 1;
-        const int64_t t0L = __shfl_sync(FULL, t0, leader); const uint64_t dtL = __shfl_sync(FULL, dtu, leader);
-        const uint32_t loL = __shfl_sync(FULL, r_lo, leader), hiL = __shfl_sync(FULL, r_hi, leader);
-        b0 = __shfl_sync(FULL, cur_b, leader);
-        const bool same = t0 == t0L && dtu == dtL && r_lo == loL && r_hi == hiL;
-        const uint32_t b_last = active ? (uint32_t)udiv_est((uint64_t)(t0 + (int64_t)r_hi * dt - q.start), (uint64_t)q.interval, inv_iv) : b0;
-        uni = __all_sync(FULL, !active || (same && b_last - b0 < OG_IL_WCAP));
-        if (uni) {
-            b_end = __reduce_max_sync(FULL, active ? b_last : 0u);
-            const uint32_t nacc = OG_IL_WCAP * q.n_calls;
-            uint8_t *base = s_acc + (size_t)wid * il_acc_bytes(q.n_calls, TIMES);
-            acc_v = (uint64_t *)base; acc_t = (int64_t *)(base + (size_t)nacc * 8); acc_k = base + (size_t)nacc * (TIMES ? 16 : 8);
-            for (uint32_t i = lane; i < nacc; i += 32) acc_k[i] = 0;
-            __syncwarp();
-        }
-    }
-    const uint32_t gcol = FOLD ? il.grp_col[grp] - ch.gc_col0 : 0;
-    const bool fold_edges = FOLD && uni && b_end > b0;
-
-    double sum = 0.0, mn = 0.0, mx = 0.0; uint64_t fi = 0, lastv = 0;
-    uint32_t n_mn = 0, n_mx = 0;
-    uint32_t w_row0 = r_lo;
-    bool head_done = false; uint32_t head_b = OG_NO_BUCKET;
-    uint32_t stop = 0, n_ev = 0;
-    auto part_of = [&](int func, uint32_t cnt) -> Part {
-        Part pp; pp.ok = cnt != 0; pp.v = 0; pp.t = 0;
-        switch (func) {
-        case OG_AGG_COUNT: pp.v = cnt; break;
-        case OG_AGG_SUM: if (FM & FM_SUM) pp.v = d2u(sum); break;
-        case OG_AGG_MIN: if (FM & FM_MIN) { pp.v = d2u(mn); if (TIMES) pp.t = t0 + (int64_t)(stop - n_mn) * dt; } break;
-        case OG_AGG_MAX: if (FM & FM_MAX) { pp.v = d2u(mx); if (TIMES) pp.t = t0 + (int64_t)(stop - n_mx) * dt; } break;
-        case OG_AGG_FIRST: if (FM & FM_FIRST) { pp.v = fi; pp.t = t0 + (int64_t)w_row0 * dt; } break;
-        default: if (FM & FM_LAST) { pp.v = lastv; pp.t = t0 + (int64_t)(stop - 1) * dt; } break;
-        }
-        return pp;
-    };
-    auto kind_of = [&]() -> int { return !head_done ? 0 : stop > r_hi ? 1 : 2; };
-    auto flush_lane = [&](int kind) {
-        const uint32_t cnt = stop - w_row0;
-#pragma unroll 1
-        for (uint32_t c = 0; c < q.n_calls; c++) {
-            const Part pp = part_of(q.calls[c].func, cnt);
-            if (kind == 2) { if (pp.ok) store_cell(ch, (int)c, series, cur_b, pp); }
-            else store_part(ch.edges[c], e + kind, pp);
-        }
-        if (kind == 0) { head_done = true; head_b = cur_b; }
-    };
-    auto flush_fold = [&](bool ev) {
-        uint32_t pend = __ballot_sync(FULL, ev);
-#pragma unroll 1
-        while (pend) {
-            const int leader = __ffs(pend) - 1;
-            const uint32_t bL = __shfl_sync(FULL, cur_b, leader);
-            const bool mine = ev && cur_b == bL;
-            const uint32_t cnt = mine ? stop - w_row0 : 0;
-            const uint32_t w = bL - b0;
-#pragma unroll 1
-            for (uint32_t c = 0; c < q.n_calls; c++) {
-                const int func = q.calls[c].func, ftype = func == OG_AGG_COUNT ? OG_TYPE_INT : q.calls[c].type;
-                const bool wt = func >= OG_AGG_MIN && !(q.multi && func <= OG_AGG_MAX);
-                Part pp = fold32(func, ftype, q.multi != 0, part_of(func, cnt), wt);
-                if ((int)lane == leader && pp.ok) {
-                    const uint32_t i = c * OG_IL_WCAP + w;
-                    Part a; a.ok = acc_k[i]; a.v = a.ok ? acc_v[i] : 0; a.t = (TIMES && a.ok) ? acc_t[i] : 0;
-                    group_update(func, ftype, q.multi != 0, a, pp);
-                    acc_v[i] = a.v; acc_k[i] = 1; if (TIMES) acc_t[i] = a.t;
-                }
-            }
-            pend &= ~__ballot_sync(FULL, mine);
-        }
-        __syncwarp();
-    };
-
-    uint32_t qp = 0, sr = 0, kfast = 0, CM = 0, CE = 0, m = 64, tr = 0, bad = 0; uint64_t MASK = 0;
-    bool done = !active;
-    uint64_t val = 0;
-
-#ifdef OG_IL_STATS
-    long long st_w0 = clock64();
-#endif
-    if (issued_b && !mbar_wait(bar0, 0)) hung = 1; else ready_b = issued_b ? 1 : 0;
-#ifdef OG_IL_STATS
-    st_wait += clock64() - st_w0;
-#endif
-    if (active && !hung) {
-        val = fetch64(col, 0); qp = 64;
-        if (lwin & OG_IL_PACKED) {
-            const uint32_t lead = (lwin >> 8) & 63u, mw = lwin & 127u;
-            qp = 64 - lead; kfast = mw;
-            MASK = mw ? (~0ull >> (64 - mw)) << (64 - lead - mw) : 0ull;
-        } else { CM = 0; CE = 1; }
-    }
-
-    bool skipping = r_lo > 0;
-    stop = skipping ? r_lo : (rb < r_hi + 1 ? rb : r_hi + 1);
-    n_ev = stop;
-    if (!skipping) { fi = val; mn = mx = u2d(val); n_mn = n_mx = n_ev; }
-    if (done) n_ev = 0xffffffffu;
-
-    auto retire = [&]() { done = true; n_ev = 0xffffffffu; CM = 0; CE = 0; MASK = 0; kfast = 0; };
-    auto advance = [&]() {
-        bool fin = false;
-        if (skipping) { skipping = false; sum = 0.0; }
-        else {
-            fin = stop > r_hi;
-            sum = 0.0;
-            if (!fin) while (stop >= rb) {
-                cur_b++;
-                rem += step_r; uint32_t adv = step_q;
-                if (rem >= dtu) { rem -= dtu; adv++; }
-                rb = (rb > 0xffffffffu - adv) ? 0xffffffffu : rb + adv;
-            }
-        }
-        if (fin) retire();
-        else {
-            w_row0 = stop;
-            uint32_t nstop = rb < r_hi + 1 ? rb : r_hi + 1;
-            n_ev = nstop - stop; stop = nstop;
-            fi = val; mn = mx = u2d(val); n_mn = n_mx = n_ev;
-        }
-    };
-    auto slow_record = [&]() {
-        uint32_t p = qp + sr;
-        const uint64_t x = fetch64(col, p);
-        const uint32_t ctrl = (uint32_t)(x >> 62);
-        if (ctrl < 2) { qp += 1; return; }
-        if (ctrl == 3) {
-            const uint32_t lm = (uint32_t)(x >> 51) & 0x7ff;
-            uint32_t lead = lm >> 6; m = lm & 0x3f;
-            if (m == 0) { m = 64; tr = 0; lead = 0; }
-            else { if (lead + m > 64) { if (!done) bad = 1; lead = 0; m = 64; } tr = 64 - lead - m; }
-            p += 13;
-            const bool slowwin = lead < 2;
-            sr = slowwin ? 0 : lead - 2;
-            CM = slowwin ? 0u : 3u << (30 - sr); CE = slowwin ? 1u : 2u << (30 - sr);
-            kfast = 2 + m;
-            MASK = (m == 64 ? ~0ull : ((1ull << m) - 1)) << tr;
-        } else p += 2;
-        const uint64_t y = fetch64(col, p);
-        const uint64_t sig = m == 64 ? y : (y >> (64 - m));
-        p += m;
-        val ^= sig << tr;
-        qp = p - sr;
-    };
-    auto accumulate = [&](uint32_t k_in_run) {
-        if (FM & FM_SUM) sum = sum + u2d(val);
-        if (FM & FM_MIN) { if (mn > u2d(val)) { mn = u2d(val); if (TIMES) n_mn = n_ev - k_in_run; } }
-        if (FM & FM_MAX) { if (mx < u2d(val)) { mx = u2d(val); if (TIMES) n_mx = n_ev - k_in_run; } }
-        if (FM & FM_LAST) lastv = val;
-    };
-    auto record = [&](uint32_t k_in_run) {
-        accumulate(k_in_run);
-        const uint64_t x = fetch64(col, qp);
-        const bool slow = (((uint32_t)(x >> 32) & CM) ^ CE) != 0;
-        if (slow) slow_record();
-        else { val ^= x & MASK; qp += kfast; }
-    };
-    auto record2 = [&](uint32_t k_in_run) {
-        const uint64_t x0 = fetch64(col, qp), x1 = fetch64(col, qp + kfast);
-        accumulate(k_in_run);
-#ifdef OG_IL_REC2B
-        uint64_t x1b = x1;
-        if ((((uint32_t)(x0 >> 32) & CM) ^ CE) != 0) { slow_record(); x1b = fetch64(col, qp); }
-        else { val ^= x0 & MASK; qp += kfast; }
-        accumulate(k_in_run + 1);
-        if ((((uint32_t)(x1b >> 32) & CM) ^ CE) != 0) slow_record();
-        else { val ^= x1b & MASK; qp += kfast; }
-#else
-        if ((((uint32_t)(x0 >> 32) & CM) ^ CE) != 0) { slow_record(); record(k_in_run + 1); return; }
-        val ^= x0 & MASK; qp += kfast;
-        accumulate(k_in_run + 1);
-        if ((((uint32_t)(x1 >> 32) & CM) ^ CE) != 0) slow_record();
-        else { val ^= x1 & MASK; qp += kfast; }
-#endif
-    };
-
-    uint32_t rounds_left = hung ? 0u : 40u * (__reduce_max_sync(FULL, rows) / K + 8u);
-#ifdef OG_IL_STATS
-    uint32_t st_common = 0, st_rare = 0, st_sit = 0, st_notgo = 0;
-    const long long st_pro = clock64() - st_clk0;
-#endif
-    for (;;) {
-        const uint32_t qmin = __reduce_min_sync(FULL, done ? 0xffffffffu : qp);
-        if (qmin == 0xffffffffu) break;
-        const uint32_t f = qmin < 32 ? 0u : (qmin - 32) >> 5;
-#pragma unroll 1
-        while (issued_b < total_b && (issued_b + 1) * B <= f + NW) { issue(issued_b); issued_b++; }
-        const uint32_t qmax = __reduce_max_sync(FULL, done ? 0u : qp);
-        uint32_t need_max = ((qmax + OG_IL_LOOKBITS) >> 5) + 1; if (need_max > rows_w) need_max = rows_w;
-        uint32_t want_b = (need_max + B - 1) / B; if (want_b > issued_b) want_b = issued_b;
-#ifdef OG_IL_STATS
-        st_w0 = clock64();
-#endif
-#pragma unroll 1
-        while (ready_b < want_b) { if (!mbar_wait(bar0 + (ready_b % NB) * 8, (ready_b / NB) & 1)) { hung = 1; break; } ready_b++; }
-#ifdef OG_IL_STATS
-        st_wait += clock64() - st_w0;
-#endif
-        if (hung) break;
-        uint32_t need = ((qp + OG_IL_LOOKBITS) >> 5) + 1; if (need > rows_w) need = rows_w;
-        bool go = done || need <= ready_b * B;
-        uint32_t run = __reduce_min_sync(FULL, go ? n_ev : 0u);
-        if (run >= K) {
-            static_assert(K % 2 == 0, "records are decoded in pairs");
-#pragma unroll UNR
-            for (uint32_t k = 0; k < K; k += 2) record2(k);
-            n_ev -= K;
-#ifdef OG_IL_STATS
-            st_common++;
-#endif
-            continue;
-        }
-#ifdef OG_IL_STATS
-        st_rare++;
-#endif
-        if (rounds_left-- == 0) { hung = 2; break; }
-        const bool all_go = __all_sync(FULL, go);
-#ifdef OG_IL_STATS
-        if (!all_go) { st_notgo++; st_sit += __popc(__ballot_sync(FULL, !go)); }
-#endif
-        uint32_t left = K;
-        for (;;) {
-            run = __reduce_min_sync(FULL, go ? n_ev : 0xffffffffu);
-            if (run > left) run = left;
-            if (all_go) {
-#pragma unroll 1
-                for (uint32_t k = 0; k < run; k++) record(k);
-            } else {
-#pragma unroll 1
-                for (uint32_t k = 0; k < run; k++) if (go) record(k);
-            }
-            if (go) n_ev -= run;
-            left -= run;
-            if (left == 0) break;
-            const bool ev = go && !done && n_ev == 0;
-            if (FOLD && uni) {
-                const bool fl = ev && !skipping;
-                const int kind = kind_of();
-                const bool to_acc = fl && (kind == 2 || fold_edges);
-                if (fl && !to_acc) flush_lane(kind);
-                if (__any_sync(FULL, to_acc)) flush_fold(to_acc);
-                if (to_acc && kind == 0) head_done = true;
-            } else if (ev && !skipping) flush_lane(kind_of());
-            if (ev) advance();
-            if (__all_sync(FULL, ev || done)) break;
-        }
-    }
-    if (active && (qp >> 5) >= rows_w) bad = 1;
-#ifdef OG_IL_STATS
-    const long long st_e0 = clock64();
-    if (lane == 0) { atomicAdd((unsigned *)&ch.err[4], st_common); atomicAdd((unsigned *)&ch.err[5], st_rare); atomicAdd((unsigned *)&ch.err[6], st_notgo); atomicAdd((unsigned *)&ch.err[7], st_sit); }
-#endif
-    while (ready_b < issued_b && hung != 1) { if (!mbar_wait(bar0 + (ready_b % NB) * 8, (ready_b / NB) & 1)) hung = 1; ready_b++; }
-    if (hung && lane == 0) report_err(ch.err, D_WATCHDOG, (grp << 2) | hung);
-    if (FOLD && uni) {
-        __syncwarp();
-        const uint32_t w_tail = fold_edges ? b_end - b0 : OG_IL_WCAP;
-        for (uint32_t i = lane; i < OG_IL_WCAP * q.n_calls; i += 32) {
-            if (!acc_k[i]) continue;
-            const uint32_t c = i / OG_IL_WCAP, w = i % OG_IL_WCAP;
-            Part a; a.ok = 1; a.v = acc_v[i]; a.t = TIMES ? acc_t[i] : 0;
-            store_part(ch.gcells[c], (size_t)(b0 + w) * ch.gc_cols + (w == w_tail ? ch.gc_tail0 + gcol : gcol), a);
-        }
-    }
-    if (FOLD && __any_sync(FULL, active && head_b != OG_NO_BUCKET) && lane == 0) ch.flags[1] = 1;
-    if (active) {
-        if (bad) report_err(ch.err, D_CORRUPT, seg);
-        *(uint2 *)(ch.edge_bucket + e) = make_uint2(head_b, (head_b == OG_NO_BUCKET || cur_b == head_b) ? OG_NO_BUCKET : cur_b);
-    }
-#ifdef OG_IL_STATS
-    if (lane == 0) {
-        atomicAdd((unsigned long long *)(ch.err + 8), (unsigned long long)st_wait);
-        const long long st_end = clock64();
-        atomicAdd((unsigned long long *)(ch.err + 10), (unsigned long long)(st_end - st_clk0));
-        atomicAdd((unsigned long long *)(ch.err + 12), (unsigned long long)st_pro);
-        atomicAdd((unsigned long long *)(ch.err + 14), (unsigned long long)(st_end - st_e0));
-    }
-#endif
-}
-
-}
+#endif
+}
+
+}
```

Measured after the change: 500.4 billion (median of 6 runs). Within noise of the previous version (-0.0%).
